# sara-nl/2D-VQ-AE-2

Measured on AMD Instinct MI355X. Metric: patches/sec (VQAE.forward: encoder -> VQ -> decoder), higher is better.
Workload: dtype f32; 1 GPU; BASELINE configs[1] (cfg B): batch 256/GPU of 256x256x3 fp32 -> 32x32 codes, K=256, D=128, full forward; global_batch=256, parallelism=patch-sharded x1

## Files before the change

2d-vq-ae-2_amd/csrc/conv_wino43.hip:

```cpp
#include "common.h"

namespace {

typedef float f32x16 __attribute__((ext_vector_type(16)));
typedef float f32x4 __attribute__((ext_vector_type(4)));
using vqae::elu_act;
using vqae::lds_barrier;

struct W43K {
    const float* __restrict__ t1;
    const float* __restrict__ U;
    const float* __restrict__ w3;
    const float* __restrict__ w1n;
    float* xio;
    float* y2;
    int H, M;
    int stag, first_gen;
    float act_a, act_b, t_scale, t_b4, n_b1a, n_b1b, n_b2a, n_b2b;
};

template <int C_> struct W43Cfg {
    static constexpr int C = C_;
    static constexpr int W = C >= 128 ? 32 : (C == 64 ? 64 : 128);
    static constexpr int NT = C == 256 ? 512 : 256;
    static constexpr int NWV = NT / 64;
    static constexpr int NS = C / 32;
    static constexpr int TG = NWV / NS;
    static constexpr int TILES = 16 * TG;
    static constexpr int TC = W / 4;
    static constexpr int PXH = 4 * W;
    static constexpr int C4 = C / 4;
    static constexpr int RP = NT / C4;
    static constexpr int LDT = C + 4;
    static constexpr int KG = C / 16;
    static constexpr int KS = C / 8;
    static constexpr int NI = C >= 64 ? 2 : 1;
    static constexpr int WN = C / (32 * NI);
    static constexpr int MI = PXH / ((NWV / WN) * 32);
    static constexpr int V_BYTES = 6 * TILES * LDT * 4, T_BYTES = PXH * LDT * 4;
    static constexpr int LDS_BYTES = V_BYTES > T_BYTES ? V_BYTES : T_BYTES;
    static_assert(TILES == 2 * TC && RP == TC && PXH / RP == 16 && MI * NI == 4, "geometry");
};
#ifndef W43_RD
#define W43_RD 4
#endif
#ifndef W43_NRES0
#define W43_NRES0 4
#endif
#ifndef W43_EARLY
#define W43_EARLY 1
#endif
constexpr int EARLY = W43_EARLY;
constexpr int RD = W43_RD;
constexpr int RT = 3;

__device__ __forceinline__ f32x4 fma4(const f32x4& a, float s, const f32x4& c) {
    return __builtin_elementwise_fma(a, f32x4{s, s, s, s}, c);
}

__device__ __forceinline__ f32x4 ldg(const float* sbase, unsigned voff_bytes) {
    return *reinterpret_cast<const f32x4*>(reinterpret_cast<const char*>(sbase) + voff_bytes);
}

#ifdef W43_TRACE
__device__ unsigned long long* g_w43_trace = nullptr;
#define STAMP(i) do { if (TAIL == 2 && lane == 0 && g_w43_trace) g_w43_trace[((int64_t)blockIdx.x * 8 + wave) * 64 + (i)] = __builtin_amdgcn_s_memtime(); } while (0)
#else
#define STAMP(i) do {} while (0)
#endif

template <int N> struct IC { static constexpr int value = N; };

template <int C, int TAIL>
__global__ __launch_bounds__((W43Cfg<C>::NT), (W43Cfg<C>::NT == 512 ? 1 : 2))
void wino43_trunk_kernel(const W43K p) {
    using K = W43Cfg<C>;
    constexpr int W = K::W, LDT = K::LDT, KG = K::KG, KS = K::KS, TILES = K::TILES, TC = K::TC, NS = K::NS, C4 = K::C4, RP = K::RP;
    constexpr int MI = K::MI, NI = K::NI, WN = K::WN;
    extern __shared__ __attribute__((aligned(16))) float lds[];
    const int tid = threadIdx.x;
    const int lane = tid & 63;
    const int wave = __builtin_amdgcn_readfirstlane(tid >> 6);
    const int li = lane & 15, q = lane >> 4;
    const int ns = wave % NS, tg = wave / NS;

    if (p.stag > 0 && (int)blockIdx.x < p.first_gen) {
        const unsigned slot = __builtin_amdgcn_s_getreg((3 << 11) | (0 << 6) | 4);
        if (slot & 1) for (int i = 0; i < p.stag; ++i) __builtin_amdgcn_s_sleep(16);
    }
#ifdef W43_TRACE
    if (TAIL == 2 && lane == 0 && g_w43_trace) {
        const unsigned hw = __builtin_amdgcn_s_getreg((15 << 11) | (0 << 6) | 4);
        const unsigned xcc = __builtin_amdgcn_s_getreg((3 << 11) | (0 << 6) | 20);
        g_w43_trace[((int64_t)blockIdx.x * 8 + wave) * 64 + 63] = ((unsigned long long)xcc << 32) | hw;
    }
#endif
    STAMP(0);
    int tile_m;
    {
        const int nwg = gridDim.x, bid = blockIdx.x;
        const int qq = nwg >> 3, r = nwg & 7, xcd = bid & 7;
        tile_m = (xcd < r ? xcd * (qq + 1) : r * (qq + 1) + (xcd - r) * qq) + (bid >> 3);
    }
    const int tpi = p.H / 8;
    const int img = tile_m / tpi;
    const int row0 = 8 * (tile_m - img * tpi);
    const float* const xim = p.t1 + (int64_t)img * p.H * W * C;

    const int cg = tid % C4, tj = tid / C4;
    unsigned coff[6];
    int roff[2][6];
#pragma unroll
    for (int j = 0; j < 6; ++j) coff[j] = (unsigned)((((4 * tj - 1 + j) & (W - 1)) * C + 4 * cg) * 4);
#pragma unroll
    for (int s = 0; s < 2; ++s)
#pragma unroll
        for (int i = 0; i < 6; ++i) {
            int r = row0 + 4 * s - 1 + i;
            r = r < 0 ? r + p.H : (r >= p.H ? r - p.H : r);
            roff[s][i] = r * W * C;
        }

    f32x4 d[2][4][2];
    f32x4 w[6];
    auto issue = [&](auto kind_c, int k) __attribute__((always_inline)) {
        constexpr int KIND = decltype(kind_c)::value;
        const int s = k / 3, cp = k % 3, bf = k & 1;
#pragma unroll
        for (int i = 0; i < (KIND == 1 ? 4 : 3); ++i) {
            const int row = KIND == 0 ? 2 * i : (KIND == 5 ? 2 * i + 1 : i + 1);
#pragma unroll
            for (int jj = 0; jj < 2; ++jj)
#ifdef W43_DBG_NOLOAD
                d[bf][i][jj] = f32x4{1.f, 2.f, (float)i, (float)tid};
#else
                d[bf][i][jj] = ldg(xim + roff[s][row], coff[2 * cp + jj]);
#endif
        }
    };
    auto combine = [&](auto kind_c, int k, float c1, float c2, float c3) __attribute__((always_inline)) {
        constexpr int KIND = decltype(kind_c)::value;
        const int cp = k % 3, bf = k & 1;
#pragma unroll
        for (int jj = 0; jj < 2; ++jj) {
            if (KIND == 1) w[2 * cp + jj] = fma4(d[bf][0][jj], c1, fma4(d[bf][1][jj], c2, fma4(d[bf][2][jj], c3, d[bf][3][jj])));
            else w[2 * cp + jj] = fma4(d[bf][0][jj], 4.f, fma4(d[bf][1][jj], -5.f, d[bf][2][jj]));
        }
    };
    auto columns = [&](int s) __attribute__((always_inline)) {
        float* const dst = lds + (s * TC + tj) * LDT + 4 * cg;
        const f32x4 t1 = fma4(w[2], -4.f, w[4]), t2 = fma4(w[1], -4.f, w[3]);
        const f32x4 t3 = w[4] - w[2], t4 = w[3] - w[1];
        *reinterpret_cast<f32x4*>(dst + 0 * TILES * LDT) = fma4(w[0], 4.f, fma4(w[2], -5.f, w[4]));
        *reinterpret_cast<f32x4*>(dst + 1 * TILES * LDT) = t1 + t2;
        *reinterpret_cast<f32x4*>(dst + 2 * TILES * LDT) = t1 - t2;
        *reinterpret_cast<f32x4*>(dst + 3 * TILES * LDT) = fma4(t4, 2.f, t3);
        *reinterpret_cast<f32x4*>(dst + 4 * TILES * LDT) = fma4(t4, -2.f, t3);
        *reinterpret_cast<f32x4*>(dst + 5 * TILES * LDT) = fma4(w[1], 4.f, fma4(w[3], -5.f, w[5]));
    };

    const float* const ub = p.U + ns * (KG * 512);
    const unsigned wl = 16u * lane;
    const float* const bfrag = lds + (16 * tg + li) * LDT + 4 * q;

    f32x4 Y[4][4][2];
#pragma unroll
    for (int a = 0; a < 4; ++a)
#pragma unroll
        for (int b = 0; b < 4; ++b) { Y[a][b][0] = f32x4{0.f, 0.f, 0.f, 0.f}; Y[a][b][1] = f32x4{0.f, 0.f, 0.f, 0.f}; }

    auto pass = [&](auto kind_c, auto next_c, int xi, float c1, float c2, float c3, float a1, float a2, float a3) __attribute__((always_inline)) {
        constexpr int KIND = decltype(kind_c)::value;
        constexpr int NEXT = decltype(next_c)::value;
        __builtin_amdgcn_sched_barrier(0);
#if defined(W43_PRIO) && W43_PRIO == 1
        __builtin_amdgcn_s_setprio(3);
#elif defined(W43_PRIO) && W43_PRIO == 2
        __builtin_amdgcn_s_setprio(0);
#endif
#pragma unroll
        for (int j = 0; j < 6; ++j) asm volatile("" : "+v"(coff[j]));
        if (EARLY < 1) issue(kind_c, 0);
#ifdef W43_SERIAL
#pragma unroll
        for (int k = 0; k < 6; ++k) {
            if (k > 0) issue(kind_c, k);
            combine(kind_c, k, c1, c2, c3);
            if (k % 3 == 2) columns(k / 3);
            __builtin_amdgcn_sched_barrier(0);
        }
#else
        if (EARLY < 2) issue(kind_c, 1);
#pragma unroll
        for (int k = 0; k < 6; ++k) {
            combine(kind_c, k, c1, c2, c3);
            if (k % 3 == 2) columns(k / 3);
            if (k + 2 < 6) issue(kind_c, k + 2);
        }
#endif
        __builtin_amdgcn_sched_barrier(0);
        int64_t uoff = (int64_t)xi * 6 * (C * C);
        asm volatile("" : "+s"(uoff));
        const float* const ux = ub + uoff;
#define WB(s) (((s) / KG) * (C * C) + 512 * ((s) % KG))
        f32x4 wq[RD][2];
#pragma unroll
        for (int s = 0; s < RD; ++s) {
            wq[s][0] = ldg(ux + WB(s), wl);
            wq[s][1] = ldg(ux + WB(s) + 256, wl);
        }
        STAMP(1 + 5 * xi);
#if defined(W43_PRIO) && W43_PRIO == 1
        __builtin_amdgcn_s_setprio(0);
#elif defined(W43_PRIO) && W43_PRIO == 2
        __builtin_amdgcn_s_setprio(3);
#endif
        lds_barrier();
        STAMP(2 + 5 * xi);
        f32x4 Z[4][2];
#pragma unroll
        for (int b = 0; b < 4; ++b) { Z[b][0] = f32x4{0.f, 0.f, 0.f, 0.f}; Z[b][1] = f32x4{0.f, 0.f, 0.f, 0.f}; }
        f32x4 acc[2][2];
        f32x4 bq[2];
        bq[0] = *reinterpret_cast<const f32x4*>(bfrag);
#pragma unroll
        for (int nu = 0; nu < 6; ++nu) {
            const int st = nu & 1;
            acc[st][0] = f32x4{0.f, 0.f, 0.f, 0.f};
            acc[st][1] = f32x4{0.f, 0.f, 0.f, 0.f};
#pragma unroll
            for (int kg = 0; kg < KG; ++kg) {
                const int s = KG * nu + kg;
                if (s + 1 < 6 * KG)
                    bq[(s + 1) & 1] = *reinterpret_cast<const f32x4*>(bfrag + ((s + 1) / KG) * TILES * LDT + 16 * ((s + 1) % KG));
                const f32x4 wa = wq[s % RD][0], wb = wq[s % RD][1];
                if (s + RD < 6 * KG) {
                    wq[s % RD][0] = ldg(ux + WB(s + RD), wl);
                    wq[s % RD][1] = ldg(ux + WB(s + RD) + 256, wl);
                }
#pragma unroll
                for (int j = 0; j < 4; ++j) {
                    acc[st][0] = __builtin_amdgcn_mfma_f32_16x16x4f32(wa[j], bq[s & 1][j], acc[st][0], 0, 0, 0);
                    acc[st][1] = __builtin_amdgcn_mfma_f32_16x16x4f32(wb[j], bq[s & 1][j], acc[st][1], 0, 0, 0);
#ifdef W43_ALT
                    __builtin_amdgcn_sched_barrier(0);
#endif
                }
                __builtin_amdgcn_sched_barrier(0);
            }
#pragma unroll
            for (int bl = 0; bl < 2; ++bl) {
                if (nu == 0) Z[0][bl] = Z[0][bl] + acc[0][bl];
                if (nu == 2) {
                    const f32x4 sm = acc[1][bl] + acc[0][bl], df = acc[1][bl] - acc[0][bl];
                    Z[0][bl] = Z[0][bl] + sm; Z[2][bl] = Z[2][bl] + sm;
                    Z[1][bl] = Z[1][bl] + df; Z[3][bl] = Z[3][bl] + df;
                }
                if (nu == 4) {
                    const f32x4 sm = acc[1][bl] + acc[0][bl], df = acc[1][bl] - acc[0][bl];
                    Z[0][bl] = Z[0][bl] + sm; Z[2][bl] = fma4(sm, 4.f, Z[2][bl]);
                    Z[1][bl] = fma4(df, 2.f, Z[1][bl]); Z[3][bl] = fma4(df, 8.f, Z[3][bl]);
                }
                if (nu == 5) Z[3][bl] = Z[3][bl] + acc[1][bl];
            }
            if (nu == 0 || nu == 2 || nu == 4)
                asm volatile("" : "+v"(Z[0][0]), "+v"(Z[0][1]), "+v"(Z[1][0]), "+v"(Z[1][1]), "+v"(Z[2][0]), "+v"(Z[2][1]), "+v"(Z[3][0]), "+v"(Z[3][1]));
        }
#undef WB
        STAMP(3 + 5 * xi);
        __builtin_amdgcn_sched_barrier(0);
        if constexpr (NEXT == 9) {
#pragma unroll
            for (int k = 0; k < EARLY; ++k)
#pragma unroll
                for (int i = 0; i < 4; ++i) {
                    const int ro = xi < 4 ? roff[0][i + 1] : roff[0][i < 3 ? 2 * i + 1 : 5];
#pragma unroll
                    for (int jj = 0; jj < 2; ++jj) d[k & 1][i][jj] = ldg(xim + ro, coff[2 * k + jj]);
                }
        } else {
            if constexpr (NEXT >= 0 && EARLY >= 1) issue(next_c, 0);
            if constexpr (NEXT >= 0 && EARLY >= 2) issue(next_c, 1);
        }
#pragma unroll
        for (int b = 0; b < 4; ++b)
#pragma unroll
            for (int bl = 0; bl < 2; ++bl) {
                if (KIND == 0) Y[0][b][bl] = Y[0][b][bl] + Z[b][bl];
                else if (KIND == 5) Y[3][b][bl] = Y[3][b][bl] + Z[b][bl];
                else {
                    Y[0][b][bl] = Y[0][b][bl] + Z[b][bl];
                    Y[1][b][bl] = fma4(Z[b][bl], a1, Y[1][b][bl]);
                    Y[2][b][bl] = fma4(Z[b][bl], a2, Y[2][b][bl]);
                    Y[3][b][bl] = fma4(Z[b][bl], a3, Y[3][b][bl]);
                }
            }
#ifdef W43_PIN_Y
#pragma unroll
        for (int a = 0; a < 4; ++a)
#pragma unroll
            for (int b = 0; b < 4; ++b) asm volatile("" : "+v"(Y[a][b][0]), "+v"(Y[a][b][1]));
#endif
        STAMP(4 + 5 * xi);
        lds_barrier();
        STAMP(5 + 5 * xi);
    };

    if (EARLY >= 1) issue(IC<0>{}, 0);
    if (EARLY >= 2) issue(IC<0>{}, 1);
    pass(IC<0>{}, IC<1>{}, 0, 0.f, 0.f, 0.f, 0.f, 0.f, 0.f);
#pragma unroll 1
    for (int xi = 1; xi <= 4; ++xi) {
        const float sg = (xi & 1) ? 1.f : -1.f;
        const bool lo = xi <= 2;
        const float c1 = lo ? -4.f * sg : -2.f * sg, c2 = lo ? -4.f : -1.f, c3 = lo ? sg : 2.f * sg;
        const float a1 = lo ? sg : 2.f * sg, a2 = lo ? 1.f : 4.f, a3 = lo ? sg : 8.f * sg;
        pass(IC<1>{}, IC<9>{}, xi, c1, c2, c3, a1, a2, a3);
    }
    pass(IC<5>{}, IC<-1>{}, 5, 0.f, 0.f, 0.f, 0.f, 0.f, 0.f);

    float* const T = lds;
    const int li32 = lane & 31, hh = lane >> 5;
    const int wm = wave / WN, wn = wave % WN;
    const int tj0 = tj;
    float* const trow = T + tj0 * LDT + 4 * cg;
    const int ty = (16 * tg + li) / TC, tx = (16 * tg + li) % TC;
    f32x4 bt[RT][NI];
    auto tail_prefetch = [&](const float* __restrict__ wsrc) __attribute__((always_inline)) {
        const float* b0 = wsrc + (wn * NI) * (KS * 256);
#pragma unroll
        for (int u = 0; u < RT; ++u)
#pragma unroll
            for (int ni = 0; ni < NI; ++ni) bt[u][ni] = ldg(b0 + ni * (KS * 256) + 256 * u, wl);
    };
    f32x16 acc[MI][NI];
    auto gemm_tail = [&](const float* __restrict__ wsrc) __attribute__((always_inline)) {
#pragma unroll
        for (int mi = 0; mi < MI; ++mi)
#pragma unroll
            for (int ni = 0; ni < NI; ++ni)
#pragma unroll
                for (int r = 0; r < 16; ++r) acc[mi][ni][r] = 0.f;
        const float* a0 = T + (wm * MI * 32 + li32) * LDT + 4 * hh;
        const float* b0 = wsrc + (wn * NI) * (KS * 256);
        f32x4 a[2][MI];
#pragma unroll
        for (int mi = 0; mi < MI; ++mi) a[0][mi] = *reinterpret_cast<const f32x4*>(a0 + mi * 32 * LDT);
#pragma unroll
        for (int ks = 0; ks < KS; ++ks) {
            if (ks + 1 < KS) {
#pragma unroll
                for (int mi = 0; mi < MI; ++mi) a[(ks + 1) & 1][mi] = *reinterpret_cast<const f32x4*>(a0 + mi * 32 * LDT + 8 * (ks + 1));
            }
            f32x4 bc[NI];
#pragma unroll
            for (int ni = 0; ni < NI; ++ni) bc[ni] = bt[ks % RT][ni];
            if (ks + RT < KS) {
#pragma unroll
                for (int ni = 0; ni < NI; ++ni) bt[ks % RT][ni] = ldg(b0 + ni * (KS * 256) + 256 * (ks + RT), wl);
            }
#pragma unroll
            for (int r = 0; r < 4; ++r)
#pragma unroll
                for (int mi = 0; mi < MI; ++mi)
#pragma unroll
                    for (int ni = 0; ni < NI; ++ni)
                        acc[mi][ni] = __builtin_amdgcn_mfma_f32_32x32x2f32(bc[ni][r], a[ks & 1][mi][r], acc[mi][ni], 0, 0, 0);
            __builtin_amdgcn_sched_barrier(0);
        }
    };
    auto acc_to_lds = [&]() __attribute__((always_inline)) {
#pragma unroll
        for (int ni = 0; ni < NI; ++ni)
#pragma unroll
            for (int mi = 0; mi < MI; ++mi)
#pragma unroll
                for (int g = 0; g < 4; ++g) {
                    f32x4 o;
#pragma unroll
                    for (int e = 0; e < 4; ++e) o[e] = acc[mi][ni][4 * g + e];
                    *reinterpret_cast<f32x4*>(T + (wm * MI * 32 + mi * 32 + li32) * LDT + (wn * NI + ni) * 32 + 8 * g + 4 * hh) = o;
                }
    };

#pragma unroll
    for (int hf = 0; hf < 2; ++hf) {
#pragma unroll
        for (int a2 = 0; a2 < 2; ++a2)
#pragma unroll
            for (int b = 0; b < 4; ++b)
#pragma unroll
                for (int bl = 0; bl < 2; ++bl) {
                    f32x4 o;
#pragma unroll
                    for (int e = 0; e < 4; ++e) o[e] = elu_act(Y[2 * hf + a2][b][bl][e] + p.act_a) + p.act_b;
                    *reinterpret_cast<f32x4*>(T + ((2 * ty + a2) * W + 4 * tx + b) * LDT + 32 * ns + 16 * bl + 4 * q) = o;
                }
        tail_prefetch(p.w3);
        const int64_t pixb = ((int64_t)img * p.H + row0 + 2 * hf) * W + tj0;
        float* xr[4];
#pragma unroll
        for (int r = 0; r < 4; ++r) xr[r] = p.xio + (pixb + (int64_t)(4 * (r >> 1) + (r & 1)) * W) * C + 4 * cg;
        f32x4 res[16];
        constexpr int NRES0 = W43_NRES0;
#pragma unroll
        for (int i = 0; i < (hf == 0 ? NRES0 : 16); ++i) res[i] = __builtin_nontemporal_load(reinterpret_cast<const f32x4*>(xr[(RP * i) / W] + ((RP * i) % W) * C));
        STAMP(31 + 8 * hf);
        lds_barrier();
        STAMP(32 + 8 * hf);
        gemm_tail(p.w3);
        STAMP(33 + 8 * hf);
        if (hf == 0) {
#pragma unroll
            for (int i = NRES0; i < 16; ++i) res[i] = __builtin_nontemporal_load(reinterpret_cast<const f32x4*>(xr[(RP * i) / W] + ((RP * i) % W) * C));
        }
        if (TAIL == 2) tail_prefetch(p.w1n);
        lds_barrier();
        acc_to_lds();
        lds_barrier();
        STAMP(34 + 8 * hf);
#pragma unroll
        for (int i = 0; i < 16; ++i) {
            f32x4 t = *reinterpret_cast<const f32x4*>(trow + RP * i * LDT);
            t = t * p.t_scale;
            t = t + p.t_b4;
            t = t + res[i];
            __builtin_nontemporal_store(t, reinterpret_cast<f32x4*>(xr[(RP * i) / W] + ((RP * i) % W) * C));
            if (TAIL == 2) {
#pragma unroll
                for (int e = 0; e < 4; ++e) t[e] = elu_act(t[e] + p.n_b1a) + p.n_b1b;
                *reinterpret_cast<f32x4*>(trow + RP * i * LDT) = t;
            }
        }
        STAMP(35 + 8 * hf);
        if constexpr (TAIL == 2) {
            lds_barrier();
            gemm_tail(p.w1n);
            STAMP(36 + 8 * hf);
            lds_barrier();
            acc_to_lds();
            lds_barrier();
            float* const y0 = p.y2 + (xr[0] - p.xio);
#pragma unroll
            for (int i = 0; i < 16; ++i) {
                f32x4 t = *reinterpret_cast<const f32x4*>(trow + RP * i * LDT);
#pragma unroll
                for (int e = 0; e < 4; ++e) t[e] = elu_act(t[e] + p.n_b2a) + p.n_b2b;
                const int r = (RP * i) / W;
                __builtin_nontemporal_store(t, reinterpret_cast<f32x4*>(y0 + ((4 * (r >> 1) + (r & 1)) * W + (RP * i) % W) * C));
            }
        }
        STAMP(37 + 8 * hf);
        if (hf == 0) lds_barrier();
        STAMP(38 + 8 * hf);
    }
}

__global__ void wino43_weight_kernel(const float* __restrict__ w, int c, float* __restrict__ U) {
    const int i = blockIdx.x * blockDim.x + threadIdx.x;
    if (i >= c * c) return;
    const double G[6][3] = {{0.25, 0, 0}, {-1.0 / 6, -1.0 / 6, -1.0 / 6}, {-1.0 / 6, 1.0 / 6, -1.0 / 6},
                            {1.0 / 24, 1.0 / 12, 1.0 / 6}, {1.0 / 24, -1.0 / 12, 1.0 / 6}, {0, 0, 1}};
    double g[3][3], t[6][3];
    for (int a = 0; a < 3; ++a)
        for (int b = 0; b < 3; ++b) g[a][b] = (double)w[(int64_t)i * 9 + a * 3 + b];
    for (int x = 0; x < 6; ++x)
        for (int b = 0; b < 3; ++b) t[x][b] = G[x][0] * g[0][b] + G[x][1] * g[1][b] + G[x][2] * g[2][b];
    const int n = i / c, k = i % c;
    const int64_t fo = ((((int64_t)(n >> 5) * (c / 16) + (k >> 4)) * 2 + ((n >> 4) & 1)) * 64 + ((k >> 2) & 3) * 16 + (n & 15)) * 4 + (k & 3);
    const int64_t cc = (int64_t)c * c;
    for (int x = 0; x < 6; ++x)
        for (int y = 0; y < 6; ++y)
            U[(x * 6 + y) * cc + fo] = (float)(t[x][0] * G[y][0] + t[x][1] * G[y][1] + t[x][2] * G[y][2]);
}

}

namespace vqae {

bool wino43_supported(int c, int h, int w, int dtype) {
    static const bool c32 = getenv("VQAE_WINO43_C32") && atoi(getenv("VQAE_WINO43_C32"));
    const bool cw = (c == 256 && w == 32) || (c == 128 && w == 32) || (c == 64 && w == 64) || (c32 && c == 32 && w == 128);
    return dtype == VQAE_DT_F32 && cw && h >= 8 && h % 8 == 0;
}
bool wino43_enabled() {
    const char* e = getenv("VQAE_WINO43");
    return !(e && !atoi(e));
}

size_t wino43_weight_floats(int c) { return (size_t)36 * c * c; }

int wino43_transform_weight(const float* w_oihw_dev, int c, float* U_dev, hipStream_t stream) {
    VQAE_REQUIRE(c == 256 || c == 128 || c == 64 || c == 32, VQAE_ERR_UNSUPPORTED, "wino43_transform_weight: C = %d", c);
    wino43_weight_kernel<<<(unsigned)ceil_div(c * c, 256), 256, 0, stream>>>(w_oihw_dev, c, U_dev);
    VQAE_LAUNCH_CHECK();
    return VQAE_OK;
}

template <int C>
static int launch_w43(W43K& k, int64_t M, bool chain, hipStream_t stream) {
    using K = W43Cfg<C>;
    static bool attr_set = false;
    static int pad = 0;
    if (!attr_set) {
#ifdef W43_TRACE
        pad = getenv("VQAE_W43_LDS_PAD") ? atoi(getenv("VQAE_W43_LDS_PAD")) : 0;
#endif
        VQAE_HIP_CHECK(hipFuncSetAttribute((const void*)wino43_trunk_kernel<C, 1>, hipFuncAttributeMaxDynamicSharedMemorySize, K::LDS_BYTES + pad));
        VQAE_HIP_CHECK(hipFuncSetAttribute((const void*)wino43_trunk_kernel<C, 2>, hipFuncAttributeMaxDynamicSharedMemorySize, K::LDS_BYTES + pad));
        attr_set = true;
    }
    const unsigned grid = (unsigned)(M / (8 * K::W));
    const double flops = 2.0 * (double)M * C * (2.25 * C + C + (chain ? C : 0));
    ProfScope prof(C >= 128 ? PROF_CONV3X3_TRUNK : PROF_NONE, stream, flops);
    if (chain) wino43_trunk_kernel<C, 2><<<grid, K::NT, K::LDS_BYTES + pad, stream>>>(k);
    else wino43_trunk_kernel<C, 1><<<grid, K::NT, K::LDS_BYTES + pad, stream>>>(k);
    prof.done();
    VQAE_LAUNCH_CHECK();
    return VQAE_OK;
}

int wino43_trunk_tail(const float* t1, const float* U, const float* w3, float act_a, float act_b, float t_scale, float t_b4,
                      float* xio, const float* w1n, float n_b1a, float n_b1b, float n_b2a, float n_b2b, float* t1_next,
                      int batch, int h, int w, int c, hipStream_t stream) {
    if (batch == 0) return VQAE_OK;
    VQAE_REQUIRE(t1 && U && w3 && xio && (!w1n || t1_next), VQAE_ERR_INVALID, "wino43_trunk_tail: null pointer");
    VQAE_REQUIRE(wino43_supported(c, h, w, VQAE_DT_F32), VQAE_ERR_UNSUPPORTED, "wino43_trunk_tail: C = %d, H = %d, W = %d", c, h, w);
    const int64_t M = (int64_t)batch * h * w;
    VQAE_REQUIRE(M < (1ll << 31) - 1024, VQAE_ERR_UNSUPPORTED, "wino43_trunk_tail: too many pixels");
    W43K k;
    memset(&k, 0, sizeof(k));
    k.t1 = t1; k.U = U; k.w3 = w3; k.w1n = w1n; k.xio = xio; k.y2 = t1_next;
    k.H = h; k.M = (int)M;
    k.act_a = act_a; k.act_b = act_b; k.t_scale = t_scale; k.t_b4 = t_b4;
    k.n_b1a = n_b1a; k.n_b1b = n_b1b; k.n_b2a = n_b2a; k.n_b2b = n_b2b;
    static const int stag = getenv("VQAE_W43_STAG") ? atoi(getenv("VQAE_W43_STAG")) : 0;
    k.stag = stag; k.first_gen = 512;
    switch (c) {
        case 256: return launch_w43<256>(k, M, w1n != nullptr, stream);
        case 128: return launch_w43<128>(k, M, w1n != nullptr, stream);
        case 64: return launch_w43<64>(k, M, w1n != nullptr, stream);
        default: return launch_w43<32>(k, M, w1n != nullptr, stream);
    }
}

}

#ifdef W43_TRACE
extern "C" int vqae_debug_w43_trace(void* dev_buf) {
    return hipMemcpyToSymbol(HIP_SYMBOL(g_w43_trace), &dev_buf, sizeof(dev_buf)) == hipSuccess ? 0 : -3;
}
#endif
```

2d-vq-ae-2_amd/csrc/handle.hip:

```cpp
#include "common.h"

#include <algorithm>
#include <cmath>
#include <cstdlib>
#include <string>
#include <unordered_map>
#include <vector>

namespace vqae {
char* last_error_buf() {
    static thread_local char buf[512] = {0};
    return buf;
}
int conv_trunk_tail(const vqae_conv_args* a, const float* t1, const float* w2, const float* w3, float t_scale,
                    float t_b4, float* xio, const float* w1n, float n_b1a, float n_b1b, float n_b2a, float n_b2b,
                    float* t1_next, hipStream_t stream);
bool wino_trunk_supported(int c, int h, int w, int dtype);
size_t wino_weight_floats(int c);
int wino_transform_weight(const float* w_oihw_dev, int c, int dtype, float* U_dev, hipStream_t stream);
int wino_frag_weight(const float* w_packed_dev, int c, int sk, float* out_dev, hipStream_t stream);
int conv_tail_kslice(int dtype, int cin);
bool wino43_supported(int c, int h, int w, int dtype);
bool wino43_enabled();
size_t wino43_weight_floats(int c);
int wino43_transform_weight(const float* w_oihw_dev, int c, float* U_dev, hipStream_t stream);
int wino43_trunk_tail(const float* t1, const float* U, const float* w3, float act_a, float act_b, float t_scale, float t_b4,
                      float* xio, const float* w1n, float n_b1a, float n_b1b, float n_b2a, float n_b2b, float* t1_next,
                      int batch, int h, int w, int c, hipStream_t stream);
int wino_trunk_tail(const float* t1, const float* U, const float* w3, float act_a, float act_b, float t_scale, float t_b4,
                    float* xio, const float* w1n, float n_b1a, float n_b1b, float n_b2a, float n_b2b, float* t1_next,
                    int batch, int h, int w, int c, int dtype, hipStream_t stream);
bool trunk16_supported(int c, int h, int w, int dtype);
size_t trunk16_weight_bytes(int c, int taps);
int trunk16_pack_weight(const float* w_packed_dev, int c, int taps, int dtype, void* out_dev, hipStream_t stream);
int trunk16_round_pack(const float* src, void* dst, int64_t n, int dtype, hipStream_t stream);
bool trunk16_head_supported(int c, int64_t m, int dtype);
int trunk16_head(const float* x, const void* w1f, float b1a, float b1b, float b2a, float b2b, void* t1, int64_t m, int c,
                 int dtype, bool out32, hipStream_t stream);
bool stem16_supported(int c0, int h, int w, int dtype);
size_t stem16_weight_bytes(int cin);
int stem16_pack_weight(const float* w_dev, int n_out, int cin, int dtype, void* out_dev, hipStream_t stream);
int istem16(const void* x, int x_kind, const float* mean255, const float* inv_std255, const void* wf, const float* bias, int B,
            int H, int W, int c0, float* y, int dtype, hipStream_t stream);
int ostem16(const float* x, const void* wf, const float* bias, int B, int H, int W, int c, float* y, int y_nchw, int dtype,
            hipStream_t stream);
bool same8_16_supported(int c, int h, int w, int dtype);
int same8_16_block(const float* x, float* y, const float* w1_packed, const void* w2h, const void* w3h, int B, int H, int W,
                   const float* scalars8, int dtype, hipStream_t stream);
bool same16_16_supported(int c, int h, int w, int dtype);
int same16_16_block(const float* x, float* y, const void* w1h, const void* w2h, const void* w3h, int B, int H, int W, int c,
                    const float* scalars8, int dtype, hipStream_t stream);
bool up16_supported(int c, int h, int w, int dtype);
int up16_block(const float* x, const float* t1, const void* w2h, const void* w3h, const void* wskh, int B, int H, int W, int c,
               float b3a, float b3b, float scale, float b4, float b1c, float b1d, int dtype, float* y, hipStream_t stream);
int trunk16_block(const void* t1, const void* w2f, const void* w3f, float act_a, float act_b, float t_scale, float t_b4,
                  float* xio, const void* w1nf, float n_b1a, float n_b1b, float n_b2a, float n_b2b, void* t1_next,
                  int batch, int h, int w, int c, int dtype, hipStream_t stream);
bool fixup_conv1_supported(int c, int64_t m);
int fixup_conv1(const float* x, const float* w1f, float pa, float pb, float aa, float ab, float* y, int64_t m, int c,
                hipStream_t stream);
bool down_block_supported(int cin, int h, int w);
int frag_weight_rect(const float* w_packed_dev, int n_rows, int K, float* out_dev, hipStream_t stream);
bool down16_supported(int cin, int h, int w);
size_t down16_weight_bytes(int n_rows, int K);
int down16_pack_weight(const float* w_packed_dev, int n_rows, int K, int dtype, void* out_dev, hipStream_t stream);
int down16_block(const float* x, const void* w1h, const void* w2h, const void* w3h, const void* wskh, int B, int H, int W,
                 int cin, const float* scalars10, int dtype, float* y, hipStream_t stream);
int down_block(const float* x, const float* w1f, const float* w2f, const float* w3f, const float* wskf, int B, int H, int W,
               int cin, const float* scalars10, int dtype, float* y, hipStream_t stream);
bool up_tail_supported(int cb, int co);
int up_tail(const float* q, const float* s, const float* w3_packed, int B, int H, int W, int cb, int co, float b3a, float b3b,
            float scale, float b4, float* y, hipStream_t stream);
int conv3x3_direct(const void* x, int x_kind, const float* mean255, const float* inv_std255, const float* w,
                   const float* bias, int B, int H, int W, int cin, int cout, float* y, int y_nchw, int dt,
                   hipStream_t stream);
}

namespace vqae {
ProfState& prof_state() {
    static ProfState p;
    return p;
}
}

extern "C" int vqae_prof_begin(int kernel_class, int max_launches) {
    vqae::ProfState& p = vqae::prof_state();
    VQAE_REQUIRE(kernel_class >= 1 && kernel_class <= 3 && max_launches >= 1, VQAE_ERR_INVALID, "prof_begin: bad args");
    if (p.cap < 2 * max_launches) {
        for (int i = 0; i < p.cap; ++i) (void)hipEventDestroy(p.ev[i]);
        delete[] p.ev;
        p.ev = new hipEvent_t[2 * max_launches];
        p.cap = 0;
        for (int i = 0; i < 2 * max_launches; ++i) {
            VQAE_HIP_CHECK(hipEventCreate(&p.ev[i]));
            p.cap = i + 1;
        }
    }
    p.used = 0;
    p.work = 0.0;
    p.cls = kernel_class;
    return VQAE_OK;
}

extern "C" int vqae_prof_end(double* total_ms, int* n_launches, double* total_work) {
    vqae::ProfState& p = vqae::prof_state();
    p.cls = 0;
    double tot = 0.0;
    for (int i = 0; i + 1 < p.used; i += 2) {
        VQAE_HIP_CHECK(hipEventSynchronize(p.ev[i + 1]));
        float ms = 0.f;
        VQAE_HIP_CHECK(hipEventElapsedTime(&ms, p.ev[i], p.ev[i + 1]));
        tot += ms;
    }
    if (total_ms) *total_ms = tot;
    if (n_launches) *n_launches = p.used / 2;
    if (total_work) *total_work = p.work;
    p.used = 0;
    return VQAE_OK;
}

extern "C" const char* vqae_last_error(void) { return vqae::last_error_buf(); }
extern "C" const char* vqae_build_info(void) { return "gfx950;fp32-mfma;" __DATE__; }

namespace {

enum { MODE_SAME = 0, MODE_DOWN = 1, MODE_UP = 2 };

struct Block {
    int mode, cin, cout, br;
    float b1a, b1b, b2a, b2b, b3a, b3b, b4, scale, b1c, b1d;
    float *w1, *w2, *w3, *wskip;
    float* wU43 = nullptr;
    float* wU = nullptr;
    float *w1f = nullptr, *w3f = nullptr;
    float *w2f = nullptr, *wskf = nullptr;
    void *w1h = nullptr, *w2h = nullptr, *w3h = nullptr;
    void *dw1h = nullptr, *dw2h = nullptr, *dw3h = nullptr, *dwskh = nullptr;
    void *uw1h = nullptr, *uw2h = nullptr, *uw3h = nullptr, *uwskh = nullptr;
    void *s8w2h = nullptr, *s8w3h = nullptr;
    int kind = VQAE_BLOCK_FIXUP, hidden = 0;
    float *bv1 = nullptr, *bv2 = nullptr, *bv3 = nullptr;
    float *fc0w = nullptr, *fc0b = nullptr, *fc2w = nullptr, *fc2b = nullptr;
};

const float kMean255[3] = {0.7279f * 255.0f, 0.5955f * 255.0f, 0.7762f * 255.0f};
const float kInv255[3] = {1.0f / (0.2419f * 255.0f), 1.0f / (0.3083f * 255.0f), 1.0f / (0.1741f * 255.0f)};

}

struct vqae_handle {
    vqae_config cfg;
    int C = 0, D = 0, K = 0;
    std::vector<Block> enc, dec;
    float *stem_w = nullptr, *stem_b = nullptr, *ostem_w = nullptr, *ostem_b = nullptr;
    void *stem_wh = nullptr, *ostem_wh = nullptr;
    bool fuse_stem16 = true;
    float *embed = nullptr;
    float *pin_w = nullptr, *pin_b = nullptr, *pout_w = nullptr, *pout_b = nullptr;
    float *pin_wt = nullptr, *pout_wr = nullptr;
    bool fuse_vq = true;
    std::vector<void*> owned;
    float* buf[4] = {nullptr, nullptr, nullptr, nullptr};
    size_t buf_floats = 0;
    void* vq_ws = nullptr;
    size_t vq_ws_bytes = 0;
    float* loss_scratch = nullptr;
    int device = 0;
    bool has_encoder = false, has_decoder = false;
    bool fuse_trunk = true;
    bool t1_ready = false;
    bool up_conv_first = true;
    bool fuse_down = true;
    bool fuse_down16 = true;
    bool fuse_up16 = true;
    bool fuse_up_tail = true;
    bool use_wino = true;
    void* idx_scratch = nullptr;
    size_t idx_scratch_bytes = 0;
    float* se_ws = nullptr;
    size_t se_ws_floats = 0;
    size_t se_gate_off = 0;
};

namespace {

using TensorMap = std::unordered_map<std::string, const vqae_tensor*>;

int find(const TensorMap& tm, const std::string& name, int64_t numel, const float** out) {
    auto it = tm.find(name);
    if (it == tm.end()) return vqae::fail(VQAE_ERR_NOT_FOUND, "missing tensor '%s'", name.c_str());
    if (it->second->numel != numel)
        return vqae::fail(VQAE_ERR_INVALID, "tensor '%s' has %lld elements, expected %lld", name.c_str(),
                          (long long)it->second->numel, (long long)numel);
    *out = it->second->data;
    return VQAE_OK;
}

int dev_alloc(vqae_handle* h, size_t bytes, void** out) {
    void* p = nullptr;
    if (hipMalloc(&p, bytes ? bytes : 16) != hipSuccess)
        return vqae::fail(VQAE_ERR_NOMEM, "hipMalloc of %zu bytes failed", bytes);
    h->owned.push_back(p);
    *out = p;
    return VQAE_OK;
}

int upload(vqae_handle* h, const float* host, int64_t numel, float** out) {
    void* p;
    int rc = dev_alloc(h, (size_t)numel * 4, &p);
    if (rc) return rc;
    VQAE_HIP_CHECK(hipMemcpy(p, host, (size_t)numel * 4, hipMemcpyHostToDevice));
    *out = (float*)p;
    return VQAE_OK;
}

int upload_packed(vqae_handle* h, const float* host, int cout, int cin, int ks, float** out) {
    float* raw = nullptr;
    void* tmp = nullptr;
    const int64_t numel = (int64_t)cout * cin * ks * ks;
    if (hipMalloc(&tmp, (size_t)numel * 4) != hipSuccess) return vqae::fail(VQAE_ERR_NOMEM, "hipMalloc failed");
    raw = (float*)tmp;
    hipError_t e = hipMemcpy(raw, host, (size_t)numel * 4, hipMemcpyHostToDevice);
    void* packed = nullptr;
    int rc = (e == hipSuccess) ? dev_alloc(h, vqae_conv_packed_floats(cout, cin, ks) * 4, &packed)
                               : vqae::fail(VQAE_ERR_HIP, "hipMemcpy failed: %s", hipGetErrorString(e));
    if (rc == VQAE_OK) rc = vqae_conv_pack_weight_f32(raw, cout, cin, ks, (float*)packed, nullptr);
    if (rc == VQAE_OK) rc = vqae_round_inplace_f32((float*)packed, (int64_t)vqae_conv_packed_floats(cout, cin, ks), h->cfg.compute_dtype, nullptr);
    if (rc == VQAE_OK && hipDeviceSynchronize() != hipSuccess) rc = vqae::fail(VQAE_ERR_HIP, "pack sync failed");
    (void)hipFree(tmp);
    *out = (float*)packed;
    return rc;
}

int upload_wino(vqae_handle* h, const float* host, int c, float** out) {
    void* tmp = nullptr;
    const size_t raw = (size_t)c * c * 9 * 4;
    if (hipMalloc(&tmp, raw) != hipSuccess) return vqae::fail(VQAE_ERR_NOMEM, "hipMalloc failed");
    hipError_t e = hipMemcpy(tmp, host, raw, hipMemcpyHostToDevice);
    void* U = nullptr;
    int rc = (e == hipSuccess) ? dev_alloc(h, vqae::wino_weight_floats(c) * 4, &U)
                               : vqae::fail(VQAE_ERR_HIP, "hipMemcpy failed: %s", hipGetErrorString(e));
    if (rc == VQAE_OK) rc = vqae::wino_transform_weight((const float*)tmp, c, h->cfg.compute_dtype, (float*)U, nullptr);
    if (rc == VQAE_OK && hipDeviceSynchronize() != hipSuccess) rc = vqae::fail(VQAE_ERR_HIP, "winograd weight transform failed");
    (void)hipFree(tmp);
    *out = (float*)U;
    return rc;
}

int upload_wino43(vqae_handle* h, const float* host, int c, float** out) {
    void* tmp = nullptr;
    const size_t raw = (size_t)c * c * 9 * 4;
    if (hipMalloc(&tmp, raw) != hipSuccess) return vqae::fail(VQAE_ERR_NOMEM, "hipMalloc failed");
    hipError_t e = hipMemcpy(tmp, host, raw, hipMemcpyHostToDevice);
    void* U = nullptr;
    int rc = (e == hipSuccess) ? dev_alloc(h, vqae::wino43_weight_floats(c) * 4, &U)
                               : vqae::fail(VQAE_ERR_HIP, "hipMemcpy failed: %s", hipGetErrorString(e));
    if (rc == VQAE_OK) rc = vqae::wino43_transform_weight((const float*)tmp, c, (float*)U, nullptr);
    if (rc == VQAE_OK && hipDeviceSynchronize() != hipSuccess) rc = vqae::fail(VQAE_ERR_HIP, "winograd weight transform failed");
    (void)hipFree(tmp);
    *out = (float*)U;
    return rc;
}

int scalar(const TensorMap& tm, const std::string& name, float* out) {
    const float* p;
    int rc = find(tm, name, 1, &p);
    if (rc) return rc;
    *out = p[0];
    return VQAE_OK;
}

int load_block(vqae_handle* h, const TensorMap& tm, const std::string& pre, int mode, int cin, int cout, Block* b) {
    b->mode = mode; b->cin = cin; b->cout = cout; b->br = cin > cout ? cin : cout;
    b->w1 = b->w2 = b->w3 = b->wskip = nullptr;
    b->b1c = b->b1d = 0.f;
    int rc;
#define S_(field, nm) if ((rc = scalar(tm, pre + "." nm, &b->field))) return rc;
    S_(b1a, "bias1a") S_(b1b, "bias1b") S_(b2a, "bias2a") S_(b2b, "bias2b") S_(b3a, "bias3a") S_(b3b, "bias3b")
    S_(b4, "bias4") S_(scale, "scale")
    const int k2 = mode == MODE_SAME ? 3 : (mode == MODE_DOWN ? 2 : 1);
    const float* p;
    if ((rc = find(tm, pre + ".branch_conv1.weight", (int64_t)b->br * cin, &p))) return rc;
    if ((rc = upload_packed(h, p, b->br, cin, 1, &b->w1))) return rc;
    if ((rc = find(tm, pre + ".branch_conv2.weight", (int64_t)b->br * b->br * k2 * k2, &p))) return rc;
    if ((rc = upload_packed(h, p, b->br, b->br, k2, &b->w2))) return rc;
    b->wU = b->wU43 = b->w1f = b->w3f = nullptr;
    const bool wino = mode == MODE_SAME && cout == cin && h->use_wino &&
                      (h->cfg.compute_dtype == VQAE_DT_F32 ? (cin == 256 || cin == 128 || cin == 64 || cin == 32) : cin == 32);
    if (wino && (rc = upload_wino(h, p, cin, &b->wU))) return rc;
    if (wino && h->cfg.compute_dtype == VQAE_DT_F32 && vqae::wino43_enabled() && vqae::wino43_supported(cin, 8, cin >= 128 ? 32 : (cin == 64 ? 64 : 128), VQAE_DT_F32) &&
        (rc = upload_wino43(h, p, cin, &b->wU43))) return rc;
    if ((rc = find(tm, pre + ".branch_conv3.weight", (int64_t)cout * b->br, &p))) return rc;
    if ((rc = upload_packed(h, p, cout, b->br, 1, &b->w3))) return rc;
    if (wino || (mode == MODE_SAME && (cin == 128 || cin == 64) && cout == cin)) {
        const int sk = wino ? 8 : vqae::conv_tail_kslice(h->cfg.compute_dtype, cin);
        void *f1, *f3;
        if ((rc = dev_alloc(h, (size_t)cin * cin * 4, &f1)) || (rc = dev_alloc(h, (size_t)cin * cin * 4, &f3))) return rc;
        b->w1f = (float*)f1; b->w3f = (float*)f3;
        if ((rc = vqae::wino_frag_weight(b->w1, cin, sk, b->w1f, nullptr)) || (rc = vqae::wino_frag_weight(b->w3, cin, sk, b->w3f, nullptr))) return rc;
        VQAE_HIP_CHECK(hipDeviceSynchronize());
    }
    b->w1h = b->w2h = b->w3h = nullptr;
    if (mode == MODE_SAME && cout == cin && h->cfg.compute_dtype != VQAE_DT_F32 && (cin == 16 || cin == 32 || cin == 64 || cin == 128 || cin == 256)) {
        struct { float* src; int taps; void** dst; } m[3] = {{b->w1, 1, &b->w1h}, {b->w2, 9, &b->w2h}, {b->w3, 1, &b->w3h}};
        for (auto& e : m) {
            if ((rc = dev_alloc(h, vqae::trunk16_weight_bytes(cin, e.taps), e.dst))) return rc;
            if ((rc = vqae::trunk16_pack_weight(e.src, cin, e.taps, h->cfg.compute_dtype, *e.dst, nullptr))) return rc;
        }
        VQAE_HIP_CHECK(hipDeviceSynchronize());
    }
    if (mode != MODE_SAME) {
        S_(b1c, "bias1c") S_(b1d, "bias1d")
        const int ks = mode == MODE_DOWN ? 2 : 1;
        if ((rc = find(tm, pre + ".skip_conv.weight", (int64_t)cout * cin * ks * ks, &p))) return rc;
        if ((rc = upload_packed(h, p, cout, cin, ks, &b->wskip))) return rc;
    }
    b->w2f = b->wskf = nullptr;
    if (mode == MODE_DOWN && h->fuse_down && cout == 2 * cin &&
        (cin == 16 || cin == 32 || cin == 64)) {
        struct { float* src; int K; float** dst; } m[4] = {{b->w1, cin, &b->w1f}, {b->w2, 4 * cout, &b->w2f},
                                                          {b->w3, cout, &b->w3f}, {b->wskip, 4 * cin, &b->wskf}};
        for (auto& e : m) {
            void* f;
            if ((rc = dev_alloc(h, (size_t)cout * e.K * 4, &f))) return rc;
            *e.dst = (float*)f;
            if ((rc = vqae::frag_weight_rect(e.src, cout, e.K, *e.dst, nullptr))) return rc;
        }
        VQAE_HIP_CHECK(hipDeviceSynchronize());
    }
    if (mode == MODE_DOWN && cout == 2 * cin && h->cfg.compute_dtype != VQAE_DT_F32 && h->fuse_down16 &&
        (cin == 8 || cin == 16 || cin == 32 || cin == 64)) {
        struct { float* src; int K; void** dst; } m16[4] = {{b->w1, cin, &b->dw1h}, {b->w2, 4 * cout, &b->dw2h},
                                                            {b->w3, cout, &b->dw3h}, {b->wskip, 4 * cin, &b->dwskh}};
        for (auto& e : m16) {
            if ((rc = dev_alloc(h, vqae::down16_weight_bytes(cout, e.K), e.dst))) return rc;
            if ((rc = vqae::down16_pack_weight(e.src, cout, e.K, h->cfg.compute_dtype, *e.dst, nullptr))) return rc;
        }
        VQAE_HIP_CHECK(hipDeviceSynchronize());
    }
    if (mode == MODE_SAME && cin == 8 && cout == 8 && h->cfg.compute_dtype != VQAE_DT_F32) {
        if ((rc = dev_alloc(h, vqae::down16_weight_bytes(8, 72), &b->s8w2h)) || (rc = dev_alloc(h, vqae::down16_weight_bytes(8, 8), &b->s8w3h))) return rc;
        if ((rc = vqae::down16_pack_weight(b->w2, 8, 72, h->cfg.compute_dtype, b->s8w2h, nullptr))) return rc;
        if ((rc = vqae::down16_pack_weight(b->w3, 8, 8, h->cfg.compute_dtype, b->s8w3h, nullptr))) return rc;
        VQAE_HIP_CHECK(hipDeviceSynchronize());
    }
    if (mode == MODE_UP && cin == 2 * cout && h->cfg.compute_dtype != VQAE_DT_F32 && h->fuse_up16 &&
        (cin == 16 || cin == 32 || cin == 64 || cin == 128)) {
        if ((rc = dev_alloc(h, vqae::trunk16_weight_bytes(cin, 1), &b->uw1h))) return rc;
        if ((rc = vqae::trunk16_pack_weight(b->w1, cin, 1, h->cfg.compute_dtype, b->uw1h, nullptr))) return rc;
        struct { float* src; int rows; void** dst; } mu[3] = {{b->w2, cin, &b->uw2h}, {b->w3, cout, &b->uw3h}, {b->wskip, cout, &b->uwskh}};
        for (auto& e : mu) {
            if ((rc = dev_alloc(h, vqae::down16_weight_bytes(e.rows, cin), e.dst))) return rc;
            if ((rc = vqae::down16_pack_weight(e.src, e.rows, cin, h->cfg.compute_dtype, *e.dst, nullptr))) return rc;
        }
        VQAE_HIP_CHECK(hipDeviceSynchronize());
    }
#undef S_
    return VQAE_OK;
}

int bn_fold(const TensorMap& tm, const std::string& pre, int c, float eps, std::vector<float>* g, std::vector<float>* shift) {
    const float *gamma, *beta, *mean, *var;
    int rc;
    if ((rc = find(tm, pre + ".weight", c, &gamma)) || (rc = find(tm, pre + ".bias", c, &beta)) ||
        (rc = find(tm, pre + ".running_mean", c, &mean)) || (rc = find(tm, pre + ".running_var", c, &var))) return rc;
    g->resize(c); shift->resize(c);
    for (int i = 0; i < c; ++i) {
        (*g)[i] = gamma[i] / std::sqrt(var[i] + eps);
        (*shift)[i] = beta[i] - mean[i] * (*g)[i];
    }
    return VQAE_OK;
}

int load_mbconv(vqae_handle* h, const TensorMap& tm, const std::string& pre, int mode, int cin, int cout, Block* b) {
    *b = Block();
    b->kind = VQAE_BLOCK_MBCONV;
    b->mode = mode; b->cin = cin; b->cout = cout;
    const int e = (cin > cout ? cin : cout) * h->cfg.expand_ratio;
    b->br = e;
    const int div = h->cfg.se_divisor;
    b->hidden = std::max(div, (int)(e + div / 2.0)) / div;
    VQAE_REQUIRE(e % 32 == 0 && e <= 1024, VQAE_ERR_UNSUPPORTED, "MBConv: expanded width %d must be a multiple of 32, <= 1024", e);
    const std::string br = pre + ".branch.";
    const float eps = h->cfg.bn_eps;
    std::vector<float> g, sh, w;
    const float* p;
    int rc;
    if ((rc = find(tm, br + "0.weight", (int64_t)e * cin, &p)) || (rc = bn_fold(tm, br + "1", e, eps, &g, &sh))) return rc;
    w.assign(p, p + (int64_t)e * cin);
    for (int o = 0; o < e; ++o) for (int i = 0; i < cin; ++i) w[(int64_t)o * cin + i] *= g[o];
    if ((rc = upload_packed(h, w.data(), e, cin, 1, &b->w1)) || (rc = upload(h, sh.data(), e, &b->bv1))) return rc;
    const int k2 = mode == MODE_SAME ? 3 : 2;
    if ((rc = find(tm, br + "3.weight", (int64_t)e * k2 * k2, &p)) || (rc = bn_fold(tm, br + "4", e, eps, &g, &sh))) return rc;
    w.assign((size_t)k2 * k2 * e, 0.f);
    for (int c = 0; c < e; ++c) for (int t = 0; t < k2 * k2; ++t) w[(size_t)t * e + c] = p[(size_t)c * k2 * k2 + t] * g[c];
    if ((rc = upload(h, w.data(), (int64_t)k2 * k2 * e, &b->w2)) || (rc = upload(h, sh.data(), e, &b->bv2))) return rc;
    if ((rc = find(tm, br + "6.fc.0.weight", (int64_t)b->hidden * e, &p)) || (rc = upload(h, p, (int64_t)b->hidden * e, &b->fc0w))) return rc;
    if ((rc = find(tm, br + "6.fc.0.bias", b->hidden, &p)) || (rc = upload(h, p, b->hidden, &b->fc0b))) return rc;
    if ((rc = find(tm, br + "6.fc.2.weight", (int64_t)e * b->hidden, &p)) || (rc = upload(h, p, (int64_t)e * b->hidden, &b->fc2w))) return rc;
    if ((rc = find(tm, br + "6.fc.2.bias", e, &p)) || (rc = upload(h, p, e, &b->fc2b))) return rc;
    if ((rc = find(tm, br + "7.weight", (int64_t)cout * e, &p)) || (rc = bn_fold(tm, br + "8", cout, eps, &g, &sh))) return rc;
    w.assign(p, p + (int64_t)cout * e);
    for (int o = 0; o < cout; ++o) for (int i = 0; i < e; ++i) w[(int64_t)o * e + i] *= g[o];
    if ((rc = upload_packed(h, w.data(), cout, e, 1, &b->w3)) || (rc = upload(h, sh.data(), cout, &b->bv3))) return rc;
    if (mode == MODE_DOWN) {
        if ((rc = find(tm, pre + ".skip_conv.weight", (int64_t)cout * cin * 4, &p)) || (rc = upload_packed(h, p, cout, cin, 2, &b->wskip))) return rc;
    } else if (mode == MODE_UP) {
        if ((rc = find(tm, pre + ".skip_conv.weight", (int64_t)cin * cout * 4, &p))) return rc;
        w.assign((size_t)4 * cout * cin, 0.f);
        for (int ci = 0; ci < cin; ++ci) for (int co = 0; co < cout; ++co) for (int t = 0; t < 4; ++t)
            w[((size_t)t * cout + co) * cin + ci] = p[((size_t)ci * cout + co) * 4 + t];
        if ((rc = upload_packed(h, w.data(), 4 * cout, cin, 1, &b->wskip))) return rc;
    } else if (cin != cout) {
        if ((rc = find(tm, pre + ".skip_conv.weight", (int64_t)cout * cin, &p)) || (rc = upload_packed(h, p, cout, cin, 1, &b->wskip))) return rc;
    }
    return VQAE_OK;
}

int load_any(vqae_handle* h, const TensorMap& tm, const std::string& pre, int mode, int cin, int cout, Block* b) {
    return h->cfg.block_kind == VQAE_BLOCK_MBCONV ? load_mbconv(h, tm, pre, mode, cin, cout, b)
                                                  : load_block(h, tm, pre, mode, cin, cout, b);
}

thread_local int g_dt = VQAE_DT_F32;
struct ConvCall {
    vqae_conv_args a;
    ConvCall(int B, int H, int W, int cin, int cout, int ks, int stride, int pad, int pad_mode, int dt = g_dt) {
        memset(&a, 0, sizeof(a));
        a.dtype = dt;
        a.batch = B; a.in_h = H; a.in_w = W; a.cin = cin; a.cout = cout;
        a.ksize = ks; a.stride = stride; a.pad = pad; a.pad_mode = pad_mode;
    }
    ConvCall& pre(int mode, float pa, float pb) { a.pre_mode = mode; a.pre_a = pa; a.pre_b = pb; return *this; }
    ConvCall& act(float aa, float ab) { a.has_act = 1; a.act_a = aa; a.act_b = ab; return *this; }
    ConvCall& scale_bias(float s, float b) { a.has_scale = 1; a.scale = s; a.bias_s = b; return *this; }
    ConvCall& bias(float b) { a.has_bias_s = 1; a.bias_s = b; return *this; }
};

int run_mbconv(vqae_handle* h, const Block& b, int B, int& H, int& W, hipStream_t st) {
    float *X = h->buf[0], *P = h->buf[1], *Q = h->buf[2], *R = h->buf[3];
    float* partial = h->se_ws;
    float* gate = h->se_ws + h->se_gate_off;
    const int E = b.br;
    int rc;
    const float* skip = X;
    int Ho = H, Wo = W;
    if (b.mode == MODE_DOWN) {
        ConvCall sk(B, H, W, b.cin, b.cout, 2, 2, 0, VQAE_PAD_NONE);
        if ((rc = vqae_conv2d_f32(&sk.a, X, b.wskip, nullptr, nullptr, R, st))) return rc;
        skip = R; Ho = H / 2; Wo = W / 2;
    } else if (b.mode == MODE_UP) {
        ConvCall sk(B, H, W, b.cin, 4 * b.cout, 1, 1, 0, VQAE_PAD_NONE);
        if ((rc = vqae_conv2d_f32(&sk.a, X, b.wskip, nullptr, nullptr, Q, st))) return rc;
        if ((rc = vqae_pixel_shuffle2_f32(Q, B, H, W, b.cout, R, st))) return rc;
        skip = R; Ho = 2 * H; Wo = 2 * W;
    } else if (b.wskip) {
        ConvCall sk(B, H, W, b.cin, b.cout, 1, 1, 0, VQAE_PAD_NONE);
        if ((rc = vqae_conv2d_f32(&sk.a, X, b.wskip, nullptr, nullptr, R, st))) return rc;
        skip = R;
    }
    ConvCall c1(B, H, W, b.cin, E, 1, 1, 0, VQAE_PAD_NONE);
    c1.a.has_act = VQAE_ACT_SILU;
    if ((rc = vqae_conv2d_f32(&c1.a, X, b.w1, b.bv1, nullptr, P, st))) return rc;
    const int dwm = b.mode == MODE_SAME ? VQAE_DW_SAME : (b.mode == MODE_DOWN ? VQAE_DW_DOWN : VQAE_DW_UP);
    if ((rc = vqae_dwconv_f32(P, b.w2, b.bv2, B, H, W, E, dwm, 1, Q, partial, st))) return rc;
    if ((rc = vqae_se_gate_f32(partial, B, Ho, Wo, E, b.fc0w, b.fc0b, b.hidden, b.fc2w, b.fc2b, gate, st))) return rc;
    ConvCall c3(B, Ho, Wo, E, b.cout, 1, 1, 0, VQAE_PAD_NONE);
    c3.a.pre_mode = VQAE_PRE_CHANNEL_GATE;
    float* out = skip == X ? X : R;
    if ((rc = vqae_conv2d_gated_f32(&c3.a, Q, gate, b.w3, b.bv3, skip, out, st))) return rc;
    if (out == R) std::swap(h->buf[0], h->buf[3]);
    H = Ho; W = Wo;
    return VQAE_OK;
}

int run_block(vqae_handle* h, const Block& b, const Block* next, int B, int& H, int& W, hipStream_t st) {
    if (b.kind == VQAE_BLOCK_MBCONV) return run_mbconv(h, b, B, H, W, st);
    float *X = h->buf[0], *P = h->buf[1], *Q = h->buf[2], *R = h->buf[3];
    int rc;
    if (b.mode == MODE_SAME && b.w2h && h->fuse_trunk && vqae::same16_16_supported(b.cin, H, W, g_dt)) {
        const float sc[8] = {b.b1a, b.b1b, b.b2a, b.b2b, b.b3a, b.b3b, b.b4, b.scale};
        if ((rc = vqae::same16_16_block(X, P, b.w1h, b.w2h, b.w3h, B, H, W, b.cin, sc, g_dt, st))) return rc;
        std::swap(h->buf[0], h->buf[1]);
        h->t1_ready = false;
        return VQAE_OK;
    }
    if (b.mode == MODE_SAME && b.w2h && h->fuse_trunk && vqae::trunk16_supported(b.cin, H, W, g_dt)) {
        if (!h->t1_ready && vqae::trunk16_head_supported(b.cin, (int64_t)B * H * W, g_dt)) {
            if ((rc = vqae::trunk16_head(X, b.w1h, b.b1a, b.b1b, b.b2a, b.b2b, P, (int64_t)B * H * W, b.cin, g_dt, false, st))) return rc;
        } else if (!h->t1_ready) {
            ConvCall c1(B, H, W, b.cin, b.br, 1, 1, 0, VQAE_PAD_NONE);
            c1.pre(VQAE_PRE_BIAS_ELU_BIAS, b.b1a, b.b1b).act(b.b2a, b.b2b);
            if ((rc = vqae_conv2d_f32(&c1.a, X, b.w1, nullptr, nullptr, Q, st))) return rc;
            if ((rc = vqae::trunk16_round_pack(Q, P, (int64_t)B * H * W * b.cin, g_dt, st))) return rc;
        }
        const bool chain = next && next->mode == MODE_SAME && next->cin == b.cin && next->cout == b.cin && next->w1h;
        if ((rc = vqae::trunk16_block(P, b.w2h, b.w3h, b.b3a, b.b3b, b.scale, b.b4, X, chain ? next->w1h : nullptr,
                                      chain ? next->b1a : 0.f, chain ? next->b1b : 0.f, chain ? next->b2a : 0.f,
                                      chain ? next->b2b : 0.f, chain ? Q : nullptr, B, H, W, b.cin, g_dt, st))) return rc;
        if (chain) std::swap(h->buf[1], h->buf[2]);
        h->t1_ready = chain;
        return VQAE_OK;
    }
    const bool wino = b.mode == MODE_SAME && b.wU && h->fuse_trunk && vqae::wino_trunk_supported(b.cin, H, W, g_dt);
    if (b.mode == MODE_SAME && (wino || ((b.cin == 128 || b.cin == 64) && b.cout == b.cin && h->fuse_trunk))) {
        if (!h->t1_ready) {
            const int64_t M = (int64_t)B * H * W;
            if (wino && g_dt == VQAE_DT_F32 && vqae::fixup_conv1_supported(b.cin, M)) {
                if ((rc = vqae::fixup_conv1(X, b.w1f, b.b1a, b.b1b, b.b2a, b.b2b, P, M, b.cin, st))) return rc;
            } else {
                ConvCall c1(B, H, W, b.cin, b.br, 1, 1, 0, VQAE_PAD_NONE);
                c1.pre(VQAE_PRE_BIAS_ELU_BIAS, b.b1a, b.b1b).act(b.b2a, b.b2b);
                if ((rc = vqae_conv2d_f32(&c1.a, X, b.w1, nullptr, nullptr, P, st))) return rc;
            }
        }
        const bool chain = next && next->mode == MODE_SAME && next->cin == b.cin && next->cout == b.cin && (!wino || next->w1f);
        if (wino && b.wU43 && vqae::wino43_supported(b.cin, H, W, g_dt)) {
            if ((rc = vqae::wino43_trunk_tail(P, b.wU43, b.w3f, b.b3a, b.b3b, b.scale, b.b4, X, chain ? next->w1f : nullptr,
                                              chain ? next->b1a : 0.f, chain ? next->b1b : 0.f, chain ? next->b2a : 0.f,
                                              chain ? next->b2b : 0.f, chain ? Q : nullptr, B, H, W, b.cin, st))) return rc;
            if (chain) std::swap(h->buf[1], h->buf[2]);
            h->t1_ready = chain;
            return VQAE_OK;
        }
        if (wino) {
            if ((rc = vqae::wino_trunk_tail(P, b.wU, b.w3f, b.b3a, b.b3b, b.scale, b.b4, X, chain ? next->w1f : nullptr,
                                            chain ? next->b1a : 0.f, chain ? next->b1b : 0.f, chain ? next->b2a : 0.f,
                                            chain ? next->b2b : 0.f, chain ? Q : nullptr, B, H, W, b.cin, g_dt, st))) return rc;
            if (chain) std::swap(h->buf[1], h->buf[2]);
            h->t1_ready = chain;
            return VQAE_OK;
        }
        ConvCall c2(B, H, W, b.br, b.br, 3, 1, 1, VQAE_PAD_CIRCULAR);
        c2.act(b.b3a, b.b3b);
        if ((rc = vqae::conv_trunk_tail(&c2.a, P, b.w2, b.w3f, b.scale, b.b4, X, chain ? next->w1f : nullptr,
                                        chain ? next->b1a : 0.f, chain ? next->b1b : 0.f, chain ? next->b2a : 0.f,
                                        chain ? next->b2b : 0.f, chain ? Q : nullptr, st))) return rc;
        if (chain) std::swap(h->buf[1], h->buf[2]);
        h->t1_ready = chain;
        return VQAE_OK;
    }
    h->t1_ready = false;
    if (b.mode == MODE_SAME && b.s8w2h && g_dt != VQAE_DT_F32 && vqae::same8_16_supported(b.cin, H, W, g_dt)) {
        const float sc[8] = {b.b1a, b.b1b, b.b2a, b.b2b, b.b3a, b.b3b, b.b4, b.scale};
        if ((rc = vqae::same8_16_block(X, P, b.w1, b.s8w2h, b.s8w3h, B, H, W, sc, g_dt, st))) return rc;
        std::swap(h->buf[0], h->buf[1]);
        return VQAE_OK;
    }
    if (b.mode == MODE_SAME && b.cin == b.cout && vqae_fixup_same_supported(b.cin, H, W)) {
        const float sc[8] = {b.b1a, b.b1b, b.b2a, b.b2b, b.b3a, b.b3b, b.b4, b.scale};
        if ((rc = vqae_fixup_same_block_f32(X, P, b.w1, b.w2, b.w3, B, H, W, b.cin, sc, g_dt, st))) return rc;
        std::swap(h->buf[0], h->buf[1]);
        return VQAE_OK;
    }
    if (b.mode == MODE_SAME) {
        ConvCall c1(B, H, W, b.cin, b.br, 1, 1, 0, VQAE_PAD_NONE);
        c1.pre(VQAE_PRE_BIAS_ELU_BIAS, b.b1a, b.b1b).act(b.b2a, b.b2b);
        if ((rc = vqae_conv2d_f32(&c1.a, X, b.w1, nullptr, nullptr, P, st))) return rc;
        ConvCall c2(B, H, W, b.br, b.br, 3, 1, 1, VQAE_PAD_CIRCULAR);
        c2.act(b.b3a, b.b3b);
        if ((rc = vqae_conv2d_f32(&c2.a, P, b.w2, nullptr, nullptr, Q, st))) return rc;
        ConvCall c3(B, H, W, b.br, b.cout, 1, 1, 0, VQAE_PAD_NONE);
        c3.scale_bias(b.scale, b.b4);
        return vqae_conv2d_f32(&c3.a, Q, b.w3, nullptr, X, X, st);
    }
    if (b.mode == MODE_DOWN && b.dw2h && g_dt != VQAE_DT_F32 && vqae::down16_supported(b.cin, H, W)) {
        const float sc[10] = {b.b1a, b.b1b, b.b2a, b.b2b, b.b3a, b.b3b, b.b4, b.scale, b.b1c, b.b1d};
        if ((rc = vqae::down16_block(X, b.dw1h, b.dw2h, b.dw3h, b.dwskh, B, H, W, b.cin, sc, g_dt, R, st))) return rc;
        H /= 2; W /= 2;
        std::swap(h->buf[0], h->buf[3]);
        return VQAE_OK;
    }
    if (b.mode == MODE_DOWN && b.w2f && vqae::down_block_supported(b.cin, H, W)) {
        const float sc[10] = {b.b1a, b.b1b, b.b2a, b.b2b, b.b3a, b.b3b, b.b4, b.scale, b.b1c, b.b1d};
        if ((rc = vqae::down_block(X, b.w1f, b.w2f, b.w3f, b.wskf, B, H, W, b.cin, sc, g_dt, R, st))) return rc;
        H /= 2; W /= 2;
        std::swap(h->buf[0], h->buf[3]);
        return VQAE_OK;
    }
    if (b.mode == MODE_DOWN) {
        ConvCall sk(B, H, W, b.cin, b.cout, 2, 2, 0, VQAE_PAD_NONE);
        sk.pre(VQAE_PRE_BIAS, b.b1c, 0.f).bias(b.b1d);
        if ((rc = vqae_conv2d_f32(&sk.a, X, b.wskip, nullptr, nullptr, R, st))) return rc;
        ConvCall c1(B, H, W, b.cin, b.br, 1, 1, 0, VQAE_PAD_NONE);
        c1.pre(VQAE_PRE_BIAS_ELU_BIAS, b.b1a, b.b1b).act(b.b2a, b.b2b);
        if ((rc = vqae_conv2d_f32(&c1.a, X, b.w1, nullptr, nullptr, P, st))) return rc;
        ConvCall c2(B, H, W, b.br, b.br, 2, 2, 0, VQAE_PAD_NONE);
        c2.act(b.b3a, b.b3b);
        if ((rc = vqae_conv2d_f32(&c2.a, P, b.w2, nullptr, nullptr, Q, st))) return rc;
        H /= 2; W /= 2;
        ConvCall c3(B, H, W, b.br, b.cout, 1, 1, 0, VQAE_PAD_NONE);
        c3.scale_bias(b.scale, b.b4);
        if ((rc = vqae_conv2d_f32(&c3.a, Q, b.w3, nullptr, R, R, st))) return rc;
        std::swap(h->buf[0], h->buf[3]);
        return VQAE_OK;
    }
    if (g_dt == VQAE_DT_F32 && h->up_conv_first) {
        ConvCall sk(B, H, W, b.cin, b.cout, 1, 1, 0, VQAE_PAD_NONE);
        sk.pre(VQAE_PRE_BIAS, b.b1c, 0.f).bias(b.b1d);
        if ((rc = vqae_conv2d_f32(&sk.a, X, b.wskip, nullptr, nullptr, Q, st))) return rc;
        if (h->fuse_up_tail && vqae::up_tail_supported(b.br, b.cout)) {
            ConvCall c1(B, H, W, b.cin, b.br, 1, 1, 0, VQAE_PAD_NONE);
            c1.pre(VQAE_PRE_BIAS_ELU_BIAS, b.b1a, b.b1b).act(b.b2a, b.b2b);
            if ((rc = vqae_conv2d_f32(&c1.a, X, b.w1, nullptr, nullptr, P, st))) return rc;
            ConvCall c2(B, H, W, b.br, b.br, 1, 1, 0, VQAE_PAD_NONE);
            if ((rc = vqae_conv2d_f32(&c2.a, P, b.w2, nullptr, nullptr, R, st))) return rc;
            if ((rc = vqae::up_tail(R, Q, b.w3, B, H, W, b.br, b.cout, b.b3a, b.b3b, b.scale, b.b4, X, st))) return rc;
            H *= 2; W *= 2;
            return VQAE_OK;
        }
        if ((rc = vqae_bicubic_up2_f32(Q, B, H, W, b.cout, 0.f, R, st))) return rc;
        ConvCall c1(B, H, W, b.cin, b.br, 1, 1, 0, VQAE_PAD_NONE);
        c1.pre(VQAE_PRE_BIAS_ELU_BIAS, b.b1a, b.b1b).act(b.b2a, b.b2b);
        if ((rc = vqae_conv2d_f32(&c1.a, X, b.w1, nullptr, nullptr, P, st))) return rc;
        ConvCall c2(B, H, W, b.br, b.br, 1, 1, 0, VQAE_PAD_NONE);
        if ((rc = vqae_conv2d_f32(&c2.a, P, b.w2, nullptr, nullptr, Q, st))) return rc;
        if ((rc = vqae_bicubic_up2_f32(Q, B, H, W, b.br, 0.f, P, st))) return rc;
        H *= 2; W *= 2;
        ConvCall c3(B, H, W, b.br, b.cout, 1, 1, 0, VQAE_PAD_NONE);
        c3.pre(VQAE_PRE_BIAS_ELU_BIAS, b.b3a, b.b3b).scale_bias(b.scale, b.b4);
        if ((rc = vqae_conv2d_f32(&c3.a, P, b.w3, nullptr, R, R, st))) return rc;
        std::swap(h->buf[0], h->buf[3]);
        return VQAE_OK;
    }
    if (b.uw2h && vqae::up16_supported(b.cin, H, W, g_dt) && vqae::trunk16_head_supported(b.cin, (int64_t)B * H * W, g_dt)) {
        if ((rc = vqae::trunk16_head(X, b.uw1h, b.b1a, b.b1b, b.b2a, b.b2b, Q, (int64_t)B * H * W, b.cin, g_dt, true, st))) return rc;
        if ((rc = vqae::up16_block(X, Q, b.uw2h, b.uw3h, b.uwskh, B, H, W, b.cin, b.b3a, b.b3b, b.scale, b.b4, b.b1c, b.b1d, g_dt, R, st))) return rc;
        H *= 2; W *= 2;
        std::swap(h->buf[0], h->buf[3]);
        return VQAE_OK;
    }
    if ((rc = vqae_bicubic_up2_f32(X, B, H, W, b.cin, b.b1c, P, st))) return rc;
    ConvCall sk(B, 2 * H, 2 * W, b.cin, b.cout, 1, 1, 0, VQAE_PAD_NONE);
    sk.bias(b.b1d);
    if ((rc = vqae_conv2d_f32(&sk.a, P, b.wskip, nullptr, nullptr, R, st))) return rc;
    ConvCall c1(B, H, W, b.cin, b.br, 1, 1, 0, VQAE_PAD_NONE);
    c1.pre(VQAE_PRE_BIAS_ELU_BIAS, b.b1a, b.b1b).act(b.b2a, b.b2b);
    if ((rc = vqae_conv2d_f32(&c1.a, X, b.w1, nullptr, nullptr, Q, st))) return rc;
    if ((rc = vqae_bicubic_up2_f32(Q, B, H, W, b.br, 0.f, P, st))) return rc;
    H *= 2; W *= 2;
    ConvCall c2(B, H, W, b.br, b.br, 1, 1, 0, VQAE_PAD_NONE);
    c2.act(b.b3a, b.b3b);
    if ((rc = vqae_conv2d_f32(&c2.a, P, b.w2, nullptr, nullptr, Q, st))) return rc;
    ConvCall c3(B, H, W, b.br, b.cout, 1, 1, 0, VQAE_PAD_NONE);
    c3.scale_bias(b.scale, b.b4);
    if ((rc = vqae_conv2d_f32(&c3.a, Q, b.w3, nullptr, R, R, st))) return rc;
    std::swap(h->buf[0], h->buf[3]);
    return VQAE_OK;
}

size_t max_floats_per_patch(const vqae_handle* h, int in_h, int in_w) {
    const size_t widen = h->cfg.block_kind == VQAE_BLOCK_MBCONV ? (size_t)h->cfg.expand_ratio : 1;
    size_t full = (size_t)in_h * in_w * (size_t)(2 * h->cfg.stem) * widen;
    size_t lat = (size_t)(in_h >> h->cfg.n_down) * (in_w >> h->cfg.n_down) * (size_t)h->C * widen;
    return full > lat ? full : lat;
}

int ensure_bufs(vqae_handle* h, size_t need) {
    if (need > h->buf_floats) {
        VQAE_HIP_CHECK(hipDeviceSynchronize());
        for (int i = 0; i < 4; ++i) {
            if (h->buf[i]) (void)hipFree(h->buf[i]);
            h->buf[i] = nullptr;
        }
        h->buf_floats = 0;
        for (int i = 0; i < 4; ++i)
            if (hipMalloc((void**)&h->buf[i], need * sizeof(float)) != hipSuccess)
                return vqae::fail(VQAE_ERR_NOMEM, "workspace hipMalloc of %zu bytes failed", need * sizeof(float));
        h->buf_floats = need;
    }
    return VQAE_OK;
}

int ensure_workspace(vqae_handle* h, int B, int in_h, int in_w) {
    int rc = ensure_bufs(h, max_floats_per_patch(h, in_h, in_w) * (size_t)(B > 0 ? B : 1));
    if (rc) return rc;
    const int64_t rows = (int64_t)B * (in_h >> h->cfg.n_down) * (in_w >> h->cfg.n_down);
    size_t vq_need = vqae_vq_workspace_bytes(rows, h->K, h->D);
    if (h->D == 8) vq_need = std::max(vq_need, vqae_vq_projected_workspace_bytes(rows));
    if (vq_need > h->vq_ws_bytes) {
        VQAE_HIP_CHECK(hipDeviceSynchronize());
        if (h->vq_ws) (void)hipFree(h->vq_ws);
        h->vq_ws = nullptr; h->vq_ws_bytes = 0;
        if (hipMalloc(&h->vq_ws, vq_need) != hipSuccess)
            return vqae::fail(VQAE_ERR_NOMEM, "vq workspace hipMalloc of %zu bytes failed", vq_need);
        h->vq_ws_bytes = vq_need;
    }
    if (h->cfg.block_kind == VQAE_BLOCK_MBCONV) {
        const int e_max = 2 * h->cfg.stem * h->cfg.expand_ratio, e_lat = h->C * h->cfg.expand_ratio;
        size_t part = vqae_dw_partial_floats(B, in_h, in_w, e_max);
        const size_t part_lat = vqae_dw_partial_floats(B, in_h >> h->cfg.n_down, in_w >> h->cfg.n_down, e_lat);
        if (part_lat > part) part = part_lat;
        for (int l = 1; l < h->cfg.n_down; ++l) {
            const size_t pl = vqae_dw_partial_floats(B, in_h >> l, in_w >> l, (2 * h->cfg.stem << l) * h->cfg.expand_ratio);
            if (pl > part) part = pl;
        }
        const size_t gate_floats = (size_t)(B > 0 ? B : 1) * (size_t)(e_lat > e_max ? e_lat : e_max);
        const size_t need_se = (size_t)vqae::round_up((int64_t)part, 64) + gate_floats;
        if (need_se > h->se_ws_floats) {
            VQAE_HIP_CHECK(hipDeviceSynchronize());
            if (h->se_ws) (void)hipFree(h->se_ws);
            h->se_ws = nullptr; h->se_ws_floats = 0;
            if (hipMalloc((void**)&h->se_ws, need_se * 4) != hipSuccess)
                return vqae::fail(VQAE_ERR_NOMEM, "SE workspace hipMalloc of %zu bytes failed", need_se * 4);
            h->se_ws_floats = need_se;
        }
        h->se_gate_off = h->se_ws_floats - gate_floats;
    }
    const size_t idx_need = (size_t)vqae::round_up(rows * 4, 256);
    if (idx_need > h->idx_scratch_bytes) {
        VQAE_HIP_CHECK(hipDeviceSynchronize());
        if (h->idx_scratch) (void)hipFree(h->idx_scratch);
        h->idx_scratch = nullptr; h->idx_scratch_bytes = 0;
        if (hipMalloc(&h->idx_scratch, idx_need) != hipSuccess)
            return vqae::fail(VQAE_ERR_NOMEM, "idx scratch hipMalloc of %zu bytes failed", idx_need);
        h->idx_scratch_bytes = idx_need;
    }
    return VQAE_OK;
}

int check_device(const vqae_handle* h) {
    int dev = -1;
    VQAE_HIP_CHECK(hipGetDevice(&dev));
    VQAE_REQUIRE(dev == h->device, VQAE_ERR_INVALID, "handle was created on HIP device %d but the current device is %d", h->device, dev);
    return VQAE_OK;
}

int check_geometry(const vqae_handle* h, int B, int in_h, int in_w) {
    const int f = 1 << h->cfg.n_down;
    if (int rc = check_device(h)) return rc;
    VQAE_REQUIRE(B >= 0, VQAE_ERR_INVALID, "negative batch");
    VQAE_REQUIRE(in_h >= f && in_w >= f && in_h % f == 0 && in_w % f == 0, VQAE_ERR_INVALID,
                 "input %dx%d must be a positive multiple of 2^n_down = %d", in_h, in_w, f);
    return VQAE_OK;
}

int run_encoder_convs(vqae_handle* h, const void* x, int x_kind, int B, int in_h, int in_w, int* zh, int* zw,
                      hipStream_t st) {
    int rc;
    if (h->stem_wh && vqae::stem16_supported(h->cfg.stem, in_h, in_w, g_dt)) {
        if ((rc = vqae::istem16(x, x_kind, kMean255, kInv255, h->stem_wh, h->stem_b, B, in_h, in_w, h->cfg.stem, h->buf[0], g_dt, st))) return rc;
    } else if ((rc = vqae::conv3x3_direct(x, x_kind, kMean255, kInv255, h->stem_w, h->stem_b, B, in_h, in_w,
                                          h->cfg.in_channels, h->cfg.stem, h->buf[0], 0, g_dt, st))) return rc;
    int H = in_h, W = in_w;
    h->t1_ready = false;
    for (size_t i = 0; i < h->enc.size(); ++i)
        if ((rc = run_block(h, h->enc[i], i + 1 < h->enc.size() ? &h->enc[i + 1] : nullptr, B, H, W, st))) return rc;
    *zh = H; *zw = W;
    return VQAE_OK;
}

int run_vq(vqae_handle* h, int B, int zh, int zw, void* idx, int idx_dtype, float* loss, hipStream_t st) {
    const int64_t rows = (int64_t)B * zh * zw;
    int rc;
    if (h->cfg.projection_dim == 8 && h->fuse_vq && h->pin_wt) {
        if ((rc = vqae_vq_projected_f32(h->buf[0], h->pin_wt, h->pin_b, h->embed, h->pout_wr, h->pout_b, rows, h->C, h->D, h->K,
                                        h->cfg.commitment_cost, g_dt, idx, idx_dtype, h->buf[1], nullptr, loss, nullptr,
                                        h->vq_ws, st))) return rc;
        std::swap(h->buf[0], h->buf[1]);
        return VQAE_OK;
    }
    if (h->cfg.projection_dim > 0) {
        ConvCall pin(B, zh, zw, h->C, h->D, 1, 1, 0, VQAE_PAD_NONE);
        if ((rc = vqae_conv2d_f32(&pin.a, h->buf[0], h->pin_w, h->pin_b, nullptr, h->buf[1], st))) return rc;
        if ((rc = vqae_vq_forward_f32(h->buf[1], h->embed, rows, h->K, h->D, h->cfg.commitment_cost, idx, idx_dtype,
                                      h->buf[2], loss, nullptr, h->vq_ws, st))) return rc;
        ConvCall pout(B, zh, zw, h->D, h->C, 1, 1, 0, VQAE_PAD_NONE);
        return vqae_conv2d_f32(&pout.a, h->buf[2], h->pout_w, h->pout_b, nullptr, h->buf[0], st);
    }
    if ((rc = vqae_vq_forward_f32(h->buf[0], h->embed, rows, h->K, h->D, h->cfg.commitment_cost, idx, idx_dtype,
                                  h->buf[1], loss, nullptr, h->vq_ws, st))) return rc;
    std::swap(h->buf[0], h->buf[1]);
    return VQAE_OK;
}

int run_decoder_convs(vqae_handle* h, int B, int qh, int qw, int layout, float* out, hipStream_t st) {
    int H = qh, W = qw, rc;
    h->t1_ready = false;
    for (size_t i = 0; i < h->dec.size(); ++i)
        if ((rc = run_block(h, h->dec[i], i + 1 < h->dec.size() ? &h->dec[i + 1] : nullptr, B, H, W, st))) return rc;
    if (h->ostem_wh && vqae::stem16_supported(h->cfg.stem, H, W, g_dt))
        return vqae::ostem16(h->buf[0], h->ostem_wh, h->ostem_b, B, H, W, h->cfg.stem, out, layout == VQAE_LAYOUT_NCHW ? 1 : 0, g_dt, st);
    return vqae::conv3x3_direct(h->buf[0], 0, nullptr, nullptr, h->ostem_w, h->ostem_b, B, H, W, h->cfg.stem,
                                h->cfg.in_channels, out, layout == VQAE_LAYOUT_NCHW ? 1 : 0, g_dt, st);
}

int export_q(vqae_handle* h, int B, int zh, int zw, int layout, float* q, hipStream_t st) {
    if (!q) return VQAE_OK;
    if (layout == VQAE_LAYOUT_NCHW) return vqae_nhwc_to_nchw_f32(h->buf[0], B, h->C, zh, zw, q, st);
    VQAE_HIP_CHECK(hipMemcpyAsync(q, h->buf[0], (size_t)B * zh * zw * h->C * 4, hipMemcpyDeviceToDevice, st));
    return VQAE_OK;
}

}

extern "C" int vqae_create(const vqae_config* cfg, const vqae_tensor* tensors, int n_tensors, vqae_handle** out) {
    VQAE_REQUIRE(cfg && tensors && out, VQAE_ERR_INVALID, "vqae_create: null pointer");
    VQAE_REQUIRE(cfg->in_channels == 3, VQAE_ERR_UNSUPPORTED, "in_channels %d (only 3)", cfg->in_channels);
    VQAE_REQUIRE(cfg->stem >= 4 && cfg->stem % 4 == 0 && cfg->stem <= 64, VQAE_ERR_UNSUPPORTED, "stem %d", cfg->stem);
    VQAE_REQUIRE(cfg->stem % 8 == 0, VQAE_ERR_UNSUPPORTED, "stem %d must be a multiple of 8", cfg->stem);
    VQAE_REQUIRE(cfg->n_down >= 1 && cfg->n_down <= 6 && cfg->n_pre >= 0 && cfg->n_post >= 0 && cfg->n_enc >= 0,
                 VQAE_ERR_INVALID, "bad depth parameters");
    VQAE_REQUIRE(cfg->num_embeddings >= 1 && cfg->num_embeddings <= 65536, VQAE_ERR_UNSUPPORTED, "num_embeddings %d",
                 cfg->num_embeddings);
    VQAE_REQUIRE(cfg->projection_dim == 0 || (cfg->projection_dim % 8 == 0), VQAE_ERR_UNSUPPORTED,
                 "projection_dim %d must be 0 or a multiple of 8", cfg->projection_dim);
    VQAE_REQUIRE(cfg->compute_dtype >= VQAE_DT_F32 && cfg->compute_dtype <= VQAE_DT_F16, VQAE_ERR_INVALID,
                 "compute_dtype %d", cfg->compute_dtype);
    VQAE_REQUIRE(cfg->block_kind == VQAE_BLOCK_FIXUP || cfg->block_kind == VQAE_BLOCK_MBCONV, VQAE_ERR_INVALID,
                 "block_kind %d", cfg->block_kind);
    if (cfg->block_kind == VQAE_BLOCK_MBCONV) {
        VQAE_REQUIRE(cfg->compute_dtype == VQAE_DT_F32, VQAE_ERR_UNSUPPORTED, "MBConv blocks run in fp32 only");
        VQAE_REQUIRE(cfg->expand_ratio >= 1 && cfg->se_divisor >= 1 && cfg->bn_eps > 0.f, VQAE_ERR_INVALID,
                     "MBConv: expand_ratio %d, se_divisor %d, bn_eps %g", cfg->expand_ratio, cfg->se_divisor, (double)cfg->bn_eps);
    }
    TensorMap tm;
    for (int i = 0; i < n_tensors; ++i) tm[tensors[i].name] = &tensors[i];

    vqae_handle* h = new vqae_handle();
    h->cfg = *cfg;
    if (hipGetDevice(&h->device) != hipSuccess) { delete h; return vqae::fail(VQAE_ERR_HIP, "hipGetDevice failed"); }
    h->fuse_trunk = !(getenv("VQAE_NO_TRUNK_FUSION") && atoi(getenv("VQAE_NO_TRUNK_FUSION")));
    h->up_conv_first = !(getenv("VQAE_NO_UP_REORDER") && atoi(getenv("VQAE_NO_UP_REORDER")));
    h->use_wino = !(getenv("VQAE_NO_WINOGRAD") && atoi(getenv("VQAE_NO_WINOGRAD")));
    h->fuse_up_tail = !(getenv("VQAE_NO_UP_TAIL_FUSION") && atoi(getenv("VQAE_NO_UP_TAIL_FUSION")));
    h->fuse_down = !(getenv("VQAE_NO_DOWN_FUSION") && atoi(getenv("VQAE_NO_DOWN_FUSION")));
    h->fuse_down16 = !(getenv("VQAE_NO_DOWN16") && atoi(getenv("VQAE_NO_DOWN16")));
    h->fuse_up16 = !(getenv("VQAE_NO_UP16") && atoi(getenv("VQAE_NO_UP16")));
    h->fuse_stem16 = !(getenv("VQAE_NO_STEM16") && atoi(getenv("VQAE_NO_STEM16")));
    h->fuse_vq = !(getenv("VQAE_NO_VQ_FUSION") && atoi(getenv("VQAE_NO_VQ_FUSION")));
    h->C = cfg->stem << cfg->n_down;
    h->D = cfg->projection_dim > 0 ? cfg->projection_dim : h->C;
    h->K = cfg->num_embeddings;
    int rc = VQAE_OK;
    const float* p;
    auto bail = [&](int code) { vqae_destroy(h); return code; };

    const bool has_enc = tm.count("encoder.in_stem.weight") > 0;
    const bool has_dec = tm.count("decoder.out_stem.weight") > 0;
    if (!has_enc && !has_dec) return bail(vqae::fail(VQAE_ERR_NOT_FOUND, "neither encoder.* nor decoder.* tensors given"));
    h->has_encoder = has_enc;
    h->has_decoder = has_dec;
    int c = cfg->stem << cfg->n_down;
    const std::string vq = "encoder.vq_layers.0.";

    if (has_enc) {
        if ((rc = find(tm, "encoder.in_stem.weight", (int64_t)cfg->stem * 3 * 9, &p)) || (rc = upload(h, p, (int64_t)cfg->stem * 27, &h->stem_w))) return bail(rc);
        if ((rc = find(tm, "encoder.in_stem.bias", cfg->stem, &p)) || (rc = upload(h, p, cfg->stem, &h->stem_b))) return bail(rc);
        if (cfg->compute_dtype != VQAE_DT_F32 && h->fuse_stem16 && cfg->in_channels == 3 && (cfg->stem == 8 || cfg->stem == 16 || cfg->stem == 32)) {
            if ((rc = dev_alloc(h, vqae::stem16_weight_bytes(3), &h->stem_wh))) return bail(rc);
            if ((rc = vqae::stem16_pack_weight(h->stem_w, cfg->stem, 3, cfg->compute_dtype, h->stem_wh, nullptr))) return bail(rc);
        }
        c = cfg->stem;
        for (int lvl = 0; lvl < cfg->n_down; ++lvl) {
            const std::string base = "encoder.down_layers.0.layers." + std::to_string(lvl) + ".layers.";
            int bi = 0;
            Block b;
            for (int i = 0; i < cfg->n_pre; ++i, ++bi) {
                if ((rc = load_any(h, tm, base + std::to_string(bi), MODE_SAME, c, c, &b))) return bail(rc);
                h->enc.push_back(b);
            }
            if ((rc = load_any(h, tm, base + std::to_string(bi), MODE_DOWN, c, 2 * c, &b))) return bail(rc);
            h->enc.push_back(b); ++bi;
            for (int i = 0; i < cfg->n_post; ++i, ++bi) {
                if ((rc = load_any(h, tm, base + std::to_string(bi), MODE_SAME, 2 * c, 2 * c, &b))) return bail(rc);
                h->enc.push_back(b);
            }
            c *= 2;
        }
        for (int i = 0; i < cfg->n_enc; ++i) {
            Block b;
            if ((rc = load_any(h, tm, "encoder.pre_enc_layers.0." + std::to_string(i), MODE_SAME, c, c, &b))) return bail(rc);
            h->enc.push_back(b);
        }
    }
    if (has_enc || tm.count(vq + "embed")) {
        if ((rc = find(tm, vq + "embed", (int64_t)h->K * h->D, &p)) || (rc = upload(h, p, (int64_t)h->K * h->D, &h->embed))) return bail(rc);
        if (cfg->projection_dim > 0) {
            if ((rc = find(tm, vq + "proj_in.weight", (int64_t)h->D * h->C, &p)) || (rc = upload_packed(h, p, h->D, h->C, 1, &h->pin_w))) return bail(rc);
            if ((rc = find(tm, vq + "proj_in.bias", h->D, &p)) || (rc = upload(h, p, h->D, &h->pin_b))) return bail(rc);
            if ((rc = vqae_round_inplace_f32(h->pin_b, h->D, cfg->compute_dtype, nullptr))) return bail(rc);
            if ((rc = find(tm, vq + "proj_out.weight", (int64_t)h->C * h->D, &p)) || (rc = upload_packed(h, p, h->C, h->D, 1, &h->pout_w))) return bail(rc);
            if ((rc = find(tm, vq + "proj_out.bias", h->C, &p)) || (rc = upload(h, p, h->C, &h->pout_b))) return bail(rc);
            if ((rc = vqae_round_inplace_f32(h->pout_b, h->C, cfg->compute_dtype, nullptr))) return bail(rc);
            if (h->D == 8) {
                std::vector<float> wt((size_t)h->C * 8);
                const float* pi = tm.at(vq + "proj_in.weight")->data;
                for (int j = 0; j < 8; ++j) for (int cc = 0; cc < h->C; ++cc) wt[(size_t)cc * 8 + j] = pi[(size_t)j * h->C + cc];
                if ((rc = upload(h, wt.data(), (int64_t)h->C * 8, &h->pin_wt)) ||
                    (rc = upload(h, tm.at(vq + "proj_out.weight")->data, (int64_t)h->C * 8, &h->pout_wr))) return bail(rc);
                if ((rc = vqae_round_inplace_f32(h->pin_wt, (int64_t)h->C * 8, cfg->compute_dtype, nullptr)) ||
                    (rc = vqae_round_inplace_f32(h->pout_wr, (int64_t)h->C * 8, cfg->compute_dtype, nullptr))) return bail(rc);
            }
        }
    }
    if (has_dec) {
        if ((rc = find(tm, "decoder.out_stem.weight", (int64_t)3 * cfg->stem * 9, &p)) || (rc = upload(h, p, (int64_t)cfg->stem * 27, &h->ostem_w))) return bail(rc);
        if ((rc = find(tm, "decoder.out_stem.bias", 3, &p)) || (rc = upload(h, p, 3, &h->ostem_b))) return bail(rc);
        if (cfg->compute_dtype != VQAE_DT_F32 && h->fuse_stem16 && cfg->in_channels == 3 && (cfg->stem == 8 || cfg->stem == 16 || cfg->stem == 32)) {
            if ((rc = dev_alloc(h, vqae::stem16_weight_bytes(cfg->stem), &h->ostem_wh))) return bail(rc);
            if ((rc = vqae::stem16_pack_weight(h->ostem_w, 3, cfg->stem, cfg->compute_dtype, h->ostem_wh, nullptr))) return bail(rc);
        }
        c = cfg->stem << cfg->n_down;
        for (int i = 0; i < cfg->n_enc; ++i) {
            Block b;
            if ((rc = load_any(h, tm, "decoder.post_enc_layers.0." + std::to_string(i), MODE_SAME, c, c, &b))) return bail(rc);
            h->dec.push_back(b);
        }
        for (int lvl = 0; lvl < cfg->n_down; ++lvl) {
            const std::string base = "decoder.up_layers.0.layers." + std::to_string(lvl) + ".layers.";
            int bi = 0;
            Block b;
            for (int i = 0; i < cfg->n_pre; ++i, ++bi) {
                if ((rc = load_any(h, tm, base + std::to_string(bi), MODE_SAME, c, c, &b))) return bail(rc);
                h->dec.push_back(b);
            }
            if ((rc = load_any(h, tm, base + std::to_string(bi), MODE_UP, c, c / 2, &b))) return bail(rc);
            h->dec.push_back(b); ++bi;
            for (int i = 0; i < cfg->n_post; ++i, ++bi) {
                if ((rc = load_any(h, tm, base + std::to_string(bi), MODE_SAME, c / 2, c / 2, &b))) return bail(rc);
                h->dec.push_back(b);
            }
            c /= 2;
        }
    }
    void* ls = nullptr;
    if ((rc = dev_alloc(h, 256, &ls))) return bail(rc);
    h->loss_scratch = (float*)ls;
    *out = h;
    return VQAE_OK;
}

extern "C" void vqae_destroy(vqae_handle* h) {
    if (!h) return;
    (void)hipDeviceSynchronize();
    for (void* p : h->owned) (void)hipFree(p);
    for (int i = 0; i < 4; ++i)
        if (h->buf[i]) (void)hipFree(h->buf[i]);
    if (h->vq_ws) (void)hipFree(h->vq_ws);
    if (h->idx_scratch) (void)hipFree(h->idx_scratch);
    if (h->se_ws) (void)hipFree(h->se_ws);
    delete h;
}

extern "C" int vqae_reserve(vqae_handle* h, int max_batch, int in_h, int in_w) {
    VQAE_REQUIRE(h, VQAE_ERR_INVALID, "null handle");
    int rc = check_geometry(h, max_batch, in_h, in_w);
    if (rc) return rc;
    return ensure_workspace(h, max_batch, in_h, in_w);
}

extern "C" int vqae_set_codebook(vqae_handle* h, const float* embed_host) {
    VQAE_REQUIRE(h && embed_host && h->embed, VQAE_ERR_INVALID, "set_codebook: null pointer / handle has no codebook");
    VQAE_HIP_CHECK(hipDeviceSynchronize());
    VQAE_HIP_CHECK(hipMemcpy(h->embed, embed_host, (size_t)h->K * h->D * 4, hipMemcpyHostToDevice));
    return VQAE_OK;
}

static int encode_impl(vqae_handle* h, const void* x, int x_kind, int B, int in_h, int in_w, void* idx, int idx_dtype,
                       float* q, int q_layout, float* loss, hipStream_t st) {
    if (h) g_dt = h->cfg.compute_dtype;
    VQAE_REQUIRE(h && x && idx, VQAE_ERR_INVALID, "vqae_encode: null pointer");
    VQAE_REQUIRE(h->has_encoder, VQAE_ERR_INVALID, "vqae_encode: handle was created without encoder.* tensors");
    int rc = check_geometry(h, B, in_h, in_w);
    if (rc) return rc;
    if (B == 0) return VQAE_OK;
    if ((rc = ensure_workspace(h, B, in_h, in_w))) return rc;
    int zh, zw;
    if ((rc = run_encoder_convs(h, x, x_kind, B, in_h, in_w, &zh, &zw, st))) return rc;
    if ((rc = run_vq(h, B, zh, zw, idx, idx_dtype, loss, st))) return rc;
    return export_q(h, B, zh, zw, q_layout, q, st);
}

extern "C" int vqae_encode(vqae_handle* h, const float* x, int B, int in_h, int in_w, int layout, void* idx,
                           int idx_dtype, float* q, float* loss, void* stream) {
    return encode_impl(h, x, layout == VQAE_LAYOUT_NCHW ? 1 : 0, B, in_h, in_w, idx, idx_dtype, q, layout, loss,
                       (hipStream_t)stream);
}

extern "C" int vqae_encode_u8(vqae_handle* h, const uint8_t* x, int B, int in_h, int in_w, void* idx, int idx_dtype,
                              float* q, int q_layout, float* loss, void* stream) {
    return encode_impl(h, x, 2, B, in_h, in_w, idx, idx_dtype, q, q_layout, loss, (hipStream_t)stream);
}

extern "C" int vqae_encode_features(vqae_handle* h, const float* x, int B, int in_h, int in_w, int layout, float* z,
                                    void* stream) {
    if (h) g_dt = h->cfg.compute_dtype;
    hipStream_t st = (hipStream_t)stream;
    VQAE_REQUIRE(h && x && z, VQAE_ERR_INVALID, "vqae_encode_features: null pointer");
    VQAE_REQUIRE(h->has_encoder, VQAE_ERR_INVALID, "vqae_encode_features: handle has no encoder");
    int rc = check_geometry(h, B, in_h, in_w);
    if (rc) return rc;
    if (B == 0) return VQAE_OK;
    if ((rc = ensure_workspace(h, B, in_h, in_w))) return rc;
    int zh, zw;
    if ((rc = run_encoder_convs(h, x, layout == VQAE_LAYOUT_NCHW ? 1 : 0, B, in_h, in_w, &zh, &zw, st))) return rc;
    if (h->cfg.projection_dim > 0) {
        ConvCall pin(B, zh, zw, h->C, h->D, 1, 1, 0, VQAE_PAD_NONE);
        return vqae_conv2d_f32(&pin.a, h->buf[0], h->pin_w, h->pin_b, nullptr, z, st);
    }
    VQAE_HIP_CHECK(hipMemcpyAsync(z, h->buf[0], (size_t)B * zh * zw * h->C * 4, hipMemcpyDeviceToDevice, st));
    return VQAE_OK;
}

extern "C" int vqae_decode(vqae_handle* h, const float* q, int B, int qh, int qw, int layout, float* out, void* stream) {
    if (h) g_dt = h->cfg.compute_dtype;
    hipStream_t st = (hipStream_t)stream;
    VQAE_REQUIRE(h && q && out, VQAE_ERR_INVALID, "vqae_decode: null pointer");
    VQAE_REQUIRE(h->has_decoder, VQAE_ERR_INVALID, "vqae_decode: handle was created without decoder.* tensors");
    VQAE_REQUIRE(B >= 0 && qh >= 1 && qw >= 1, VQAE_ERR_INVALID, "vqae_decode: bad shape");
    if (int rcd = check_device(h)) return rcd;
    if (B == 0) return VQAE_OK;
    int rc;
    if ((rc = ensure_workspace(h, B, qh << h->cfg.n_down, qw << h->cfg.n_down))) return rc;
    if (layout == VQAE_LAYOUT_NCHW) {
        if ((rc = vqae_nchw_to_nhwc_f32(q, B, h->C, qh, qw, h->buf[0], st))) return rc;
    } else {
        VQAE_HIP_CHECK(hipMemcpyAsync(h->buf[0], q, (size_t)B * qh * qw * h->C * 4, hipMemcpyDeviceToDevice, st));
    }
    return run_decoder_convs(h, B, qh, qw, layout, out, st);
}

extern "C" int vqae_decode_indices(vqae_handle* h, const void* idx, int idx_dtype, int B, int qh, int qw, int layout,
                                   float* out, void* stream) {
    if (h) g_dt = h->cfg.compute_dtype;
    hipStream_t st = (hipStream_t)stream;
    VQAE_REQUIRE(h && idx && out, VQAE_ERR_INVALID, "vqae_decode_indices: null pointer");
    VQAE_REQUIRE(h->has_decoder && h->embed, VQAE_ERR_INVALID, "vqae_decode_indices: handle needs decoder.* tensors and a codebook");
    VQAE_REQUIRE(B >= 0 && qh >= 1 && qw >= 1, VQAE_ERR_INVALID, "vqae_decode_indices: bad shape");
    if (int rcd = check_device(h)) return rcd;
    if (B == 0) return VQAE_OK;
    int rc;
    if ((rc = ensure_workspace(h, B, qh << h->cfg.n_down, qw << h->cfg.n_down))) return rc;
    const int64_t rows = (int64_t)B * qh * qw;
    if (h->cfg.projection_dim > 0) {
        if ((rc = vqae_embed_code_f32(idx, idx_dtype, h->embed, rows, h->K, h->D, h->buf[1], st))) return rc;
        ConvCall pout(B, qh, qw, h->D, h->C, 1, 1, 0, VQAE_PAD_NONE);
        if ((rc = vqae_conv2d_f32(&pout.a, h->buf[1], h->pout_w, h->pout_b, nullptr, h->buf[0], st))) return rc;
    } else {
        if ((rc = vqae_embed_code_f32(idx, idx_dtype, h->embed, rows, h->K, h->D, h->buf[0], st))) return rc;
    }
    return run_decoder_convs(h, B, qh, qw, layout, out, st);
}

extern "C" int vqae_block_count(const vqae_handle* h, int side) {
    if (!h) return 0;
    return (int)(side == 0 ? h->enc.size() : h->dec.size());
}

extern "C" int vqae_run_blocks(vqae_handle* h, int side, int first, int count, const float* x, int B, int in_h, int in_w,
                               float* y, int* out_h, int* out_w, void* stream) {
    if (h) g_dt = h->cfg.compute_dtype;
    hipStream_t st = (hipStream_t)stream;
    VQAE_REQUIRE(h && x && y, VQAE_ERR_INVALID, "vqae_run_blocks: null pointer");
    VQAE_REQUIRE(side == 0 || side == 1, VQAE_ERR_INVALID, "vqae_run_blocks: side %d", side);
    std::vector<Block>& v = side == 0 ? h->enc : h->dec;
    VQAE_REQUIRE(first >= 0 && count >= 1 && (size_t)first + (size_t)count <= v.size(), VQAE_ERR_INVALID,
                 "vqae_run_blocks: blocks [%d, %d) of %zu", first, first + count, v.size());
    VQAE_REQUIRE(B >= 0 && in_h >= 1 && in_w >= 1, VQAE_ERR_INVALID, "vqae_run_blocks: bad shape");
    if (int rcd = check_device(h)) return rcd;
    int H = in_h, W = in_w;
    if (B == 0) return VQAE_OK;
    size_t need = 0;
    {
        double hh = in_h, ww = in_w;
        for (int i = first; i < first + count; ++i) {
            const Block& b = v[i];
            VQAE_REQUIRE(b.mode != MODE_DOWN || (((int)hh % 2 == 0) && ((int)ww % 2 == 0)), VQAE_ERR_INVALID,
                         "vqae_run_blocks: odd input size at a 'down' block");
            const size_t wide = (size_t)std::max(std::max(b.cin, b.cout), b.br) * (b.mode == MODE_UP ? 4 : 1);
            need = std::max(need, (size_t)B * (size_t)hh * (size_t)ww * wide);
            if (b.mode == MODE_DOWN) { hh /= 2; ww /= 2; } else if (b.mode == MODE_UP) { hh *= 2; ww *= 2; }
        }
    }
    int rc;
    if ((rc = ensure_bufs(h, need))) return rc;
    if (h->cfg.block_kind == VQAE_BLOCK_MBCONV)
        return vqae::fail(VQAE_ERR_UNSUPPORTED, "vqae_run_blocks: Fixup blocks only");
    VQAE_HIP_CHECK(hipMemcpyAsync(h->buf[0], x, (size_t)B * in_h * in_w * v[first].cin * 4, hipMemcpyDeviceToDevice, st));
    h->t1_ready = false;
    for (int i = first; i < first + count; ++i)
        if ((rc = run_block(h, v[i], i + 1 < first + count ? &v[i + 1] : nullptr, B, H, W, st))) return rc;
    h->t1_ready = false;
    VQAE_HIP_CHECK(hipMemcpyAsync(y, h->buf[0], (size_t)B * H * W * v[first + count - 1].cout * 4, hipMemcpyDeviceToDevice, st));
    if (out_h) *out_h = H;
    if (out_w) *out_w = W;
    return VQAE_OK;
}

extern "C" int vqae_forward(vqae_handle* h, const float* x, int B, int in_h, int in_w, int layout, float* out, void* idx,
                            int idx_dtype, float* loss, void* stream) {
    if (h) g_dt = h->cfg.compute_dtype;
    hipStream_t st = (hipStream_t)stream;
    VQAE_REQUIRE(h && x && out, VQAE_ERR_INVALID, "vqae_forward: null pointer");
    VQAE_REQUIRE(h->has_encoder && h->has_decoder, VQAE_ERR_INVALID, "vqae_forward: handle needs encoder.* and decoder.* tensors");
    int rc = check_geometry(h, B, in_h, in_w);
    if (rc) return rc;
    if (B == 0) return VQAE_OK;
    if ((rc = ensure_workspace(h, B, in_h, in_w))) return rc;
    int zh, zw;
    if ((rc = run_encoder_convs(h, x, layout == VQAE_LAYOUT_NCHW ? 1 : 0, B, in_h, in_w, &zh, &zw, st))) return rc;
    void* idx_out = idx;
    int dt = idx_dtype;
    if (!idx_out) { idx_out = h->idx_scratch; dt = VQAE_IDX_I32; }
    if ((rc = run_vq(h, B, zh, zw, idx_out, dt, loss ? loss : h->loss_scratch, st))) return rc;
    return run_decoder_convs(h, B, zh, zw, layout, out, st);
}

extern "C" double vqae_flops_per_patch(const vqae_handle* h, int in_h, int in_w, int encoder, int decoder) {
    if (!h) return 0.0;
    double fl = 0.0;
    auto blocks = [&](const std::vector<Block>& v, double H, double W) {
        for (const Block& b : v) {
            if (b.kind == VQAE_BLOCK_MBCONV) {
                const double k2 = b.mode == MODE_SAME ? 9.0 : 4.0;
                fl += 2.0 * H * W * (double)b.cin * b.br;
                if (b.mode == MODE_DOWN) {
                    fl += 2.0 * (H / 2) * (W / 2) * (k2 * b.br + (double)b.br * b.cout + 4.0 * b.cin * b.cout);
                    H /= 2; W /= 2;
                } else if (b.mode == MODE_UP) {
                    fl += 2.0 * H * W * 4.0 * b.cin * b.cout;
                    H *= 2; W *= 2;
                    fl += 2.0 * H * W * ((double)b.br + (double)b.br * b.cout);
                } else {
                    fl += 2.0 * H * W * (k2 * b.br + (double)b.br * b.cout + (b.wskip ? (double)b.cin * b.cout : 0.0));
                }
                continue;
            }
            if (b.mode == MODE_SAME) {
                fl += 2.0 * H * W * ((double)b.cin * b.br + 9.0 * b.br * b.br + (double)b.br * b.cout);
            } else if (b.mode == MODE_DOWN) {
                fl += 2.0 * H * W * (double)b.cin * b.br;
                H /= 2; W /= 2;
                fl += 2.0 * H * W * (4.0 * b.br * b.br + (double)b.br * b.cout + 4.0 * b.cin * b.cout);
            } else {
                fl += 2.0 * H * W * (double)b.cin * b.br;
                H *= 2; W *= 2;
                fl += 2.0 * H * W * ((double)b.br * b.br + (double)b.br * b.cout + (double)b.cin * b.cout);
            }
        }
        return std::pair<double, double>(H, W);
    };
    if (encoder) {
        fl += 2.0 * in_h * in_w * 27.0 * h->cfg.stem;
        auto hw = blocks(h->enc, in_h, in_w);
        if (h->cfg.projection_dim > 0) fl += 2.0 * hw.first * hw.second * 2.0 * h->C * h->D;
    }
    if (decoder) {
        blocks(h->dec, in_h >> h->cfg.n_down, in_w >> h->cfg.n_down);
        fl += 2.0 * in_h * in_w * 27.0 * h->cfg.stem;
    }
    return fl;
}
```

Baseline: 4101 patches/s.

## Emulate fp32 Winograd trunk GEMMs with 3-way bf16 split MFMA at C=128

Adds a split-precision path for the C=128 Winograd F(4,3) trunk kernel. Activations and weights are decomposed into three bf16 planes (hi/mid/lo) and multiplied with bf16 MFMA instructions using six cross-products, replacing the fp32 16x16x4 and 32x32x2-style MFMAs in both the Winograd-domain GEMM and the fused 1x1 tail GEMMs. Pre-split weight copies are generated at load time and the feature is on by default. This trades higher-throughput bf16 matrix ops for extra conversion ALU work and a different LDS layout, while aiming to keep near-fp32 accuracy.

```diff
diff --git a/2d-vq-ae-2_amd/csrc/conv_wino43.hip b/2d-vq-ae-2_amd/csrc/conv_wino43.hip
--- a/2d-vq-ae-2_amd/csrc/conv_wino43.hip
+++ b/2d-vq-ae-2_amd/csrc/conv_wino43.hip
@@ -4,6 +4,8 @@
 
 typedef float f32x16 __attribute__((ext_vector_type(16)));
 typedef float f32x4 __attribute__((ext_vector_type(4)));
+typedef __bf16 bf16x4 __attribute__((ext_vector_type(4)));
+typedef __bf16 bf16x8 __attribute__((ext_vector_type(8)));
 using vqae::elu_act;
 using vqae::lds_barrier;
 
@@ -14,6 +16,9 @@
     const float* __restrict__ w1n;
     float* xio;
     float* y2;
+    const float* __restrict__ Us;
+    const float* __restrict__ w3s;
+    const float* __restrict__ w1ns;
     int H, M;
     int stag, first_gen;
     float act_a, act_b, t_scale, t_b4, n_b1a, n_b1b, n_b2a, n_b2b;
@@ -39,6 +44,9 @@
     static constexpr int MI = PXH / ((NWV / WN) * 32);
     static constexpr int V_BYTES = 6 * TILES * LDT * 4, T_BYTES = PXH * LDT * 4;
     static constexpr int LDS_BYTES = V_BYTES > T_BYTES ? V_BYTES : T_BYTES;
+    static constexpr int LDVB = 3 * C + 8, KC = C / 32, KS2 = C / 16;
+    static constexpr int VS_BYTES = 6 * TILES * LDVB * 2;
+    static constexpr int LDS_SPLIT = VS_BYTES > T_BYTES ? VS_BYTES : T_BYTES;
     static_assert(TILES == 2 * TC && RP == TC && PXH / RP == 16 && MI * NI == 4, "geometry");
 };
 #ifndef W43_RD
@@ -53,6 +61,15 @@
 constexpr int EARLY = W43_EARLY;
 constexpr int RD = W43_RD;
 constexpr int RT = 3;
+
+__device__ __forceinline__ void split3(const f32x4& v, bf16x4 (&h)[3]) {
+    h[0] = __builtin_convertvector(v, bf16x4);
+    const f32x4 r1 = v - __builtin_convertvector(h[0], f32x4);
+    h[1] = __builtin_convertvector(r1, bf16x4);
+    const f32x4 r2 = r1 - __builtin_convertvector(h[1], f32x4);
+    h[2] = __builtin_convertvector(r2, bf16x4);
+}
+__device__ __forceinline__ bf16x8 as_bf8(const f32x4& v) { return __builtin_bit_cast(bf16x8, v); }
 
 __device__ __forceinline__ f32x4 fma4(const f32x4& a, float s, const f32x4& c) {
     return __builtin_elementwise_fma(a, f32x4{s, s, s, s}, c);
@@ -71,12 +88,13 @@
 
 template <int N> struct IC { static constexpr int value = N; };
 
-template <int C, int TAIL>
+template <int C, int TAIL, bool SPLIT>
 __global__ __launch_bounds__((W43Cfg<C>::NT), (W43Cfg<C>::NT == 512 ? 1 : 2))
 void wino43_trunk_kernel(const W43K p) {
     using K = W43Cfg<C>;
     constexpr int W = K::W, LDT = K::LDT, KG = K::KG, KS = K::KS, TILES = K::TILES, TC = K::TC, NS = K::NS, C4 = K::C4, RP = K::RP;
     constexpr int MI = K::MI, NI = K::NI, WN = K::WN;
+    constexpr int LDVB = K::LDVB, KC = K::KC, KS2 = K::KS2;
     extern __shared__ __attribute__((aligned(16))) float lds[];
     const int tid = threadIdx.x;
     const int lane = tid & 63;
@@ -149,17 +167,30 @@
     };
     auto columns = [&](int s) __attribute__((always_inline)) {
         float* const dst = lds + (s * TC + tj) * LDT + 4 * cg;
+        __bf16* const dsb = reinterpret_cast<__bf16*>(lds) + (s * TC + tj) * LDVB + 4 * cg;
+        auto put = [&](int nu, const f32x4& v) __attribute__((always_inline)) {
+            if constexpr (SPLIT) {
+                bf16x4 h[3];
+                split3(v, h);
+#pragma unroll
+                for (int pl = 0; pl < 3; ++pl) *reinterpret_cast<bf16x4*>(dsb + nu * TILES * LDVB + pl * C) = h[pl];
+            } else {
+                *reinterpret_cast<f32x4*>(dst + nu * TILES * LDT) = v;
+            }
+        };
         const f32x4 t1 = fma4(w[2], -4.f, w[4]), t2 = fma4(w[1], -4.f, w[3]);
         const f32x4 t3 = w[4] - w[2], t4 = w[3] - w[1];
-        *reinterpret_cast<f32x4*>(dst + 0 * TILES * LDT) = fma4(w[0], 4.f, fma4(w[2], -5.f, w[4]));
-        *reinterpret_cast<f32x4*>(dst + 1 * TILES * LDT) = t1 + t2;
-        *reinterpret_cast<f32x4*>(dst + 2 * TILES * LDT) = t1 - t2;
-        *reinterpret_cast<f32x4*>(dst + 3 * TILES * LDT) = fma4(t4, 2.f, t3);
-        *reinterpret_cast<f32x4*>(dst + 4 * TILES * LDT) = fma4(t4, -2.f, t3);
-        *reinterpret_cast<f32x4*>(dst + 5 * TILES * LDT) = fma4(w[1], 4.f, fma4(w[3], -5.f, w[5]));
+        put(0, fma4(w[0], 4.f, fma4(w[2], -5.f, w[4])));
+        put(1, t1 + t2);
+        put(2, t1 - t2);
+        put(3, fma4(t4, 2.f, t3));
+        put(4, fma4(t4, -2.f, t3));
+        put(5, fma4(w[1], 4.f, fma4(w[3], -5.f, w[5])));
     };
 
     const float* const ub = p.U + ns * (KG * 512);
+    const float* const ubs = p.Us + ns * (KC * 1536);
+    const __bf16* const vbs = reinterpret_cast<const __bf16*>(lds) + (16 * tg + li) * LDVB + 8 * q;
     const unsigned wl = 16u * lane;
     const float* const bfrag = lds + (16 * tg + li) * LDT + 4 * q;
 
@@ -199,55 +230,9 @@
         }
 #endif
         __builtin_amdgcn_sched_barrier(0);
-        int64_t uoff = (int64_t)xi * 6 * (C * C);
-        asm volatile("" : "+s"(uoff));
-        const float* const ux = ub + uoff;
-#define WB(s) (((s) / KG) * (C * C) + 512 * ((s) % KG))
-        f32x4 wq[RD][2];
-#pragma unroll
-        for (int s = 0; s < RD; ++s) {
-            wq[s][0] = ldg(ux + WB(s), wl);
-            wq[s][1] = ldg(ux + WB(s) + 256, wl);
-        }
-        STAMP(1 + 5 * xi);
-#if defined(W43_PRIO) && W43_PRIO == 1
-        __builtin_amdgcn_s_setprio(0);
-#elif defined(W43_PRIO) && W43_PRIO == 2
-        __builtin_amdgcn_s_setprio(3);
-#endif
-        lds_barrier();
-        STAMP(2 + 5 * xi);
         f32x4 Z[4][2];
-#pragma unroll
-        for (int b = 0; b < 4; ++b) { Z[b][0] = f32x4{0.f, 0.f, 0.f, 0.f}; Z[b][1] = f32x4{0.f, 0.f, 0.f, 0.f}; }
         f32x4 acc[2][2];
-        f32x4 bq[2];
-        bq[0] = *reinterpret_cast<const f32x4*>(bfrag);
-#pragma unroll
-        for (int nu = 0; nu < 6; ++nu) {
-            const int st = nu & 1;
-            acc[st][0] = f32x4{0.f, 0.f, 0.f, 0.f};
-            acc[st][1] = f32x4{0.f, 0.f, 0.f, 0.f};
-#pragma unroll
-            for (int kg = 0; kg < KG; ++kg) {
-                const int s = KG * nu + kg;
-                if (s + 1 < 6 * KG)
-                    bq[(s + 1) & 1] = *reinterpret_cast<const f32x4*>(bfrag + ((s + 1) / KG) * TILES * LDT + 16 * ((s + 1) % KG));
-                const f32x4 wa = wq[s % RD][0], wb = wq[s % RD][1];
-                if (s + RD < 6 * KG) {
-                    wq[s % RD][0] = ldg(ux + WB(s + RD), wl);
-                    wq[s % RD][1] = ldg(ux + WB(s + RD) + 256, wl);
-                }
-#pragma unroll
-                for (int j = 0; j < 4; ++j) {
-                    acc[st][0] = __builtin_amdgcn_mfma_f32_16x16x4f32(wa[j], bq[s & 1][j], acc[st][0], 0, 0, 0);
-                    acc[st][1] = __builtin_amdgcn_mfma_f32_16x16x4f32(wb[j], bq[s & 1][j], acc[st][1], 0, 0, 0);
-#ifdef W43_ALT
-                    __builtin_amdgcn_sched_barrier(0);
-#endif
-                }
-                __builtin_amdgcn_sched_barrier(0);
-            }
+        auto fold_nu = [&](int nu) __attribute__((always_inline)) {
 #pragma unroll
             for (int bl = 0; bl < 2; ++bl) {
                 if (nu == 0) Z[0][bl] = Z[0][bl] + acc[0][bl];
@@ -265,8 +250,108 @@
             }
             if (nu == 0 || nu == 2 || nu == 4)
                 asm volatile("" : "+v"(Z[0][0]), "+v"(Z[0][1]), "+v"(Z[1][0]), "+v"(Z[1][1]), "+v"(Z[2][0]), "+v"(Z[2][1]), "+v"(Z[3][0]), "+v"(Z[3][1]));
-        }
+        };
+        if constexpr (SPLIT) {
+            int64_t uoff = (int64_t)xi * 6 * (3 * C * C / 2);
+            asm volatile("" : "+s"(uoff));
+            const float* const ux = ubs + uoff;
+#define WS(s, bl, pl) (((s) / KC) * (3 * C * C / 2) + 1536 * ((s) % KC) + 256 * (3 * (bl) + (pl)))
+#define VB(s, pl) (*reinterpret_cast<const bf16x8*>(vbs + ((s) / KC) * TILES * LDVB + (pl) * C + 32 * ((s) % KC)))
+            f32x4 w0[2][2], w1[2], w2[2];
+#pragma unroll
+            for (int bl = 0; bl < 2; ++bl) {
+                w0[0][bl] = ldg(ux + WS(0, bl, 0), wl);
+                w1[bl] = ldg(ux + WS(0, bl, 1), wl);
+                w2[bl] = ldg(ux + WS(0, bl, 2), wl);
+                w0[1][bl] = ldg(ux + WS(1, bl, 0), wl);
+            }
+            STAMP(1 + 5 * xi);
+            lds_barrier();
+            STAMP(2 + 5 * xi);
+#pragma unroll
+            for (int b = 0; b < 4; ++b) { Z[b][0] = f32x4{0.f, 0.f, 0.f, 0.f}; Z[b][1] = f32x4{0.f, 0.f, 0.f, 0.f}; }
+            bf16x8 vb0 = VB(0, 0), vb1 = VB(0, 1), vb2 = VB(0, 2);
+#pragma unroll
+            for (int nu = 0; nu < 6; ++nu) {
+                const int st = nu & 1;
+                acc[st][0] = f32x4{0.f, 0.f, 0.f, 0.f};
+                acc[st][1] = f32x4{0.f, 0.f, 0.f, 0.f};
+#pragma unroll
+                for (int kc = 0; kc < KC; ++kc) {
+                    const int s = KC * nu + kc, sl = s & 1;
+                    const bool nxt = s + 1 < 6 * KC;
+#define MM(wa, vb) for (int bl = 0; bl < 2; ++bl) acc[st][bl] = __builtin_amdgcn_mfma_f32_16x16x32_bf16(as_bf8(wa[bl]), vb, acc[st][bl], 0, 0, 0)
+                    MM(w1, vb1);
+                    MM(w1, vb0);
+                    if (nxt) for (int bl = 0; bl < 2; ++bl) w1[bl] = ldg(ux + WS(s + 1, bl, 1), wl);
+                    MM(w2, vb0);
+                    if (nxt) for (int bl = 0; bl < 2; ++bl) w2[bl] = ldg(ux + WS(s + 1, bl, 2), wl);
+                    MM(w0[sl], vb2);
+                    if (nxt) vb2 = VB(s + 1, 2);
+                    MM(w0[sl], vb1);
+                    if (nxt) vb1 = VB(s + 1, 1);
+                    MM(w0[sl], vb0);
+                    if (s + 2 < 6 * KC) for (int bl = 0; bl < 2; ++bl) w0[sl][bl] = ldg(ux + WS(s + 2, bl, 0), wl);
+                    if (nxt) vb0 = VB(s + 1, 0);
+#undef MM
+                    __builtin_amdgcn_sched_barrier(0);
+                }
+                fold_nu(nu);
+            }
+#undef WS
+#undef VB
+        } else {
+            int64_t uoff = (int64_t)xi * 6 * (C * C);
+            asm volatile("" : "+s"(uoff));
+            const float* const ux = ub + uoff;
+#define WB(s) (((s) / KG) * (C * C) + 512 * ((s) % KG))
+            f32x4 wq[RD][2];
+#pragma unroll
+            for (int s = 0; s < RD; ++s) {
+                wq[s][0] = ldg(ux + WB(s), wl);
+                wq[s][1] = ldg(ux + WB(s) + 256, wl);
+            }
+            STAMP(1 + 5 * xi);
+#if defined(W43_PRIO) && W43_PRIO == 1
+            __builtin_amdgcn_s_setprio(0);
+#elif defined(W43_PRIO) && W43_PRIO == 2
+            __builtin_amdgcn_s_setprio(3);
+#endif
+            lds_barrier();
+            STAMP(2 + 5 * xi);
+#pragma unroll
+            for (int b = 0; b < 4; ++b) { Z[b][0] = f32x4{0.f, 0.f, 0.f, 0.f}; Z[b][1] = f32x4{0.f, 0.f, 0.f, 0.f}; }
+            f32x4 bq[2];
+            bq[0] = *reinterpret_cast<const f32x4*>(bfrag);
+#pragma unroll
+            for (int nu = 0; nu < 6; ++nu) {
+                const int st = nu & 1;
+                acc[st][0] = f32x4{0.f, 0.f, 0.f, 0.f};
+                acc[st][1] = f32x4{0.f, 0.f, 0.f, 0.f};
+#pragma unroll
+                for (int kg = 0; kg < KG; ++kg) {
+                    const int s = KG * nu + kg;
+                    if (s + 1 < 6 * KG)
+                        bq[(s + 1) & 1] = *reinterpret_cast<const f32x4*>(bfrag + ((s + 1) / KG) * TILES * LDT + 16 * ((s + 1) % KG));
+                    const f32x4 wa = wq[s % RD][0], wb = wq[s % RD][1];
+                    if (s + RD < 6 * KG) {
+                        wq[s % RD][0] = ldg(ux + WB(s + RD), wl);
+                        wq[s % RD][1] = ldg(ux + WB(s + RD) + 256, wl);
+                    }
+#pragma unroll
+                    for (int j = 0; j < 4; ++j) {
+                        acc[st][0] = __builtin_amdgcn_mfma_f32_16x16x4f32(wa[j], bq[s & 1][j], acc[st][0], 0, 0, 0);
+                        acc[st][1] = __builtin_amdgcn_mfma_f32_16x16x4f32(wb[j], bq[s & 1][j], acc[st][1], 0, 0, 0);
+#ifdef W43_ALT
+                        __builtin_amdgcn_sched_barrier(0);
+#endif
+                    }
+                    __builtin_amdgcn_sched_barrier(0);
+                }
+                fold_nu(nu);
+            }
 #undef WB
+        }
         STAMP(3 + 5 * xi);
         __builtin_amdgcn_sched_barrier(0);
         if constexpr (NEXT == 9) {
@@ -326,7 +411,19 @@
     float* const trow = T + tj0 * LDT + 4 * cg;
     const int ty = (16 * tg + li) / TC, tx = (16 * tg + li) % TC;
     f32x4 bt[RT][NI];
+    f32x4 bs0[2][NI], bs1[NI], bs2[NI];
     auto tail_prefetch = [&](const float* __restrict__ wsrc) __attribute__((always_inline)) {
+        if constexpr (SPLIT) {
+            const float* b0 = wsrc + (wn * NI) * (KS2 * 768);
+#pragma unroll
+            for (int ni = 0; ni < NI; ++ni) {
+                bs0[0][ni] = ldg(b0 + ni * (KS2 * 768), wl);
+                bs1[ni] = ldg(b0 + ni * (KS2 * 768) + 256, wl);
+                bs2[ni] = ldg(b0 + ni * (KS2 * 768) + 512, wl);
+                bs0[1][ni] = ldg(b0 + ni * (KS2 * 768) + 768, wl);
+            }
+            return;
+        }
         const float* b0 = wsrc + (wn * NI) * (KS * 256);
 #pragma unroll
         for (int u = 0; u < RT; ++u)
@@ -334,6 +431,38 @@
             for (int ni = 0; ni < NI; ++ni) bt[u][ni] = ldg(b0 + ni * (KS * 256) + 256 * u, wl);
     };
     f32x16 acc[MI][NI];
+    auto gemm_tail_split = [&](const float* __restrict__ wsrc) __attribute__((always_inline)) {
+        const float* a0 = T + (wm * MI * 32 + li32) * LDT + 8 * hh;
+        const float* b0 = wsrc + (wn * NI) * (KS2 * 768);
+#pragma unroll
+        for (int ks = 0; ks < KS2; ++ks) {
+            const int sl = ks & 1;
+            bf16x8 x[MI][3];
+#pragma unroll
+            for (int mi = 0; mi < MI; ++mi) {
+                bf16x4 lo[3], hi[3];
+                split3(*reinterpret_cast<const f32x4*>(a0 + mi * 32 * LDT + 16 * ks), lo);
+                split3(*reinterpret_cast<const f32x4*>(a0 + mi * 32 * LDT + 16 * ks + 4), hi);
+#pragma unroll
+                for (int pl = 0; pl < 3; ++pl) x[mi][pl] = __builtin_shufflevector(lo[pl], hi[pl], 0, 1, 2, 3, 4, 5, 6, 7);
+            }
+#define MM(wa, pb) for (int mi = 0; mi < MI; ++mi) for (int ni = 0; ni < NI; ++ni) \
+                acc[mi][ni] = __builtin_amdgcn_mfma_f32_32x32x16_bf16(as_bf8(wa[ni]), x[mi][pb], acc[mi][ni], 0, 0, 0)
+#define RELOAD(dst, k, pl) for (int ni = 0; ni < NI; ++ni) dst[ni] = ldg(b0 + ni * (KS2 * 768) + 768 * (k) + 256 * (pl), wl)
+            MM(bs1, 1);
+            MM(bs1, 0);
+            if (ks + 1 < KS2) RELOAD(bs1, ks + 1, 1);
+            MM(bs2, 0);
+            if (ks + 1 < KS2) RELOAD(bs2, ks + 1, 2);
+            MM(bs0[sl], 2);
+            MM(bs0[sl], 1);
+            MM(bs0[sl], 0);
+            if (ks + 2 < KS2) RELOAD(bs0[sl], ks + 2, 0);
+#undef MM
+#undef RELOAD
+            __builtin_amdgcn_sched_barrier(0);
+        }
+    };
     auto gemm_tail = [&](const float* __restrict__ wsrc) __attribute__((always_inline)) {
 #pragma unroll
         for (int mi = 0; mi < MI; ++mi)
@@ -341,6 +470,10 @@
             for (int ni = 0; ni < NI; ++ni)
 #pragma unroll
                 for (int r = 0; r < 16; ++r) acc[mi][ni][r] = 0.f;
+        if constexpr (SPLIT) {
+            gemm_tail_split(wsrc);
+            return;
+        }
         const float* a0 = T + (wm * MI * 32 + li32) * LDT + 4 * hh;
         const float* b0 = wsrc + (wn * NI) * (KS * 256);
         f32x4 a[2][MI];
@@ -396,7 +529,7 @@
                     for (int e = 0; e < 4; ++e) o[e] = elu_act(Y[2 * hf + a2][b][bl][e] + p.act_a) + p.act_b;
                     *reinterpret_cast<f32x4*>(T + ((2 * ty + a2) * W + 4 * tx + b) * LDT + 32 * ns + 16 * bl + 4 * q) = o;
                 }
-        tail_prefetch(p.w3);
+        tail_prefetch(SPLIT ? p.w3s : p.w3);
         const int64_t pixb = ((int64_t)img * p.H + row0 + 2 * hf) * W + tj0;
         float* xr[4];
 #pragma unroll
@@ -408,13 +541,13 @@
         STAMP(31 + 8 * hf);
         lds_barrier();
         STAMP(32 + 8 * hf);
-        gemm_tail(p.w3);
+        gemm_tail(SPLIT ? p.w3s : p.w3);
         STAMP(33 + 8 * hf);
         if (hf == 0) {
 #pragma unroll
             for (int i = NRES0; i < 16; ++i) res[i] = __builtin_nontemporal_load(reinterpret_cast<const f32x4*>(xr[(RP * i) / W] + ((RP * i) % W) * C));
         }
-        if (TAIL == 2) tail_prefetch(p.w1n);
+        if (TAIL == 2) tail_prefetch(SPLIT ? p.w1ns : p.w1n);
         lds_barrier();
         acc_to_lds();
         lds_barrier();
@@ -435,7 +568,7 @@
         STAMP(35 + 8 * hf);
         if constexpr (TAIL == 2) {
             lds_barrier();
-            gemm_tail(p.w1n);
+            gemm_tail(SPLIT ? p.w1ns : p.w1n);
             STAMP(36 + 8 * hf);
             lds_barrier();
             acc_to_lds();
@@ -456,22 +589,59 @@
     }
 }
 
-__global__ void wino43_weight_kernel(const float* __restrict__ w, int c, float* __restrict__ U) {
-    const int i = blockIdx.x * blockDim.x + threadIdx.x;
-    if (i >= c * c) return;
+__device__ void wino43_u(const float* __restrict__ w, int64_t i, double (&u)[36]) {
     const double G[6][3] = {{0.25, 0, 0}, {-1.0 / 6, -1.0 / 6, -1.0 / 6}, {-1.0 / 6, 1.0 / 6, -1.0 / 6},
                             {1.0 / 24, 1.0 / 12, 1.0 / 6}, {1.0 / 24, -1.0 / 12, 1.0 / 6}, {0, 0, 1}};
     double g[3][3], t[6][3];
     for (int a = 0; a < 3; ++a)
-        for (int b = 0; b < 3; ++b) g[a][b] = (double)w[(int64_t)i * 9 + a * 3 + b];
+        for (int b = 0; b < 3; ++b) g[a][b] = (double)w[i * 9 + a * 3 + b];
     for (int x = 0; x < 6; ++x)
         for (int b = 0; b < 3; ++b) t[x][b] = G[x][0] * g[0][b] + G[x][1] * g[1][b] + G[x][2] * g[2][b];
+    for (int x = 0; x < 6; ++x)
+        for (int y = 0; y < 6; ++y) u[x * 6 + y] = t[x][0] * G[y][0] + t[x][1] * G[y][1] + t[x][2] * G[y][2];
+}
+
+__global__ void wino43_weight_kernel(const float* __restrict__ w, int c, float* __restrict__ U) {
+    const int i = blockIdx.x * blockDim.x + threadIdx.x;
+    if (i >= c * c) return;
+    double u[36];
+    wino43_u(w, i, u);
     const int n = i / c, k = i % c;
     const int64_t fo = ((((int64_t)(n >> 5) * (c / 16) + (k >> 4)) * 2 + ((n >> 4) & 1)) * 64 + ((k >> 2) & 3) * 16 + (n & 15)) * 4 + (k & 3);
     const int64_t cc = (int64_t)c * c;
-    for (int x = 0; x < 6; ++x)
-        for (int y = 0; y < 6; ++y)
-            U[(x * 6 + y) * cc + fo] = (float)(t[x][0] * G[y][0] + t[x][1] * G[y][1] + t[x][2] * G[y][2]);
+    for (int x = 0; x < 36; ++x) U[x * cc + fo] = (float)u[x];
+}
+
+__device__ void split3_f64(double v, __bf16 (&h)[3]) {
+    for (int pl = 0; pl < 3; ++pl) {
+        h[pl] = (__bf16)(float)v;
+        v -= (double)(float)h[pl];
+    }
+}
+
+__global__ void wino43_split_weight_kernel(const float* __restrict__ w, int c, __bf16* __restrict__ U) {
+    const int i = blockIdx.x * blockDim.x + threadIdx.x;
+    if (i >= c * c) return;
+    double u[36];
+    wino43_u(w, i, u);
+    const int n = i / c, k = i % c;
+    const int64_t fo = (((int64_t)(n >> 5) * (c / 32) + (k >> 5)) * 2 + ((n >> 4) & 1)) * 3 * 512 + (((k >> 3) & 3) * 16 + (n & 15)) * 8 + (k & 7);
+    const int64_t cc = (int64_t)c * c;
+    for (int x = 0; x < 36; ++x) {
+        __bf16 h[3];
+        split3_f64(u[x], h);
+        for (int pl = 0; pl < 3; ++pl) U[x * 3 * cc + fo + pl * 512] = h[pl];
+    }
+}
+
+__global__ void split_1x1_kernel(const float* __restrict__ w, int c, __bf16* __restrict__ out) {
+    const int i = blockIdx.x * blockDim.x + threadIdx.x;
+    if (i >= c * c) return;
+    const int n = i / c, k = i % c;
+    __bf16 h[3];
+    split3_f64((double)w[i], h);
+    const int64_t fo = ((int64_t)(n >> 5) * (c / 16) + (k >> 4)) * 3 * 512 + (((k >> 3) & 1) * 32 + (n & 31)) * 8 + (k & 7);
+    for (int pl = 0; pl < 3; ++pl) out[fo + pl * 512] = h[pl];
 }
 
 }
@@ -489,6 +659,24 @@
 }
 
 size_t wino43_weight_floats(int c) { return (size_t)36 * c * c; }
+
+bool wino43_split_supported(int c) { return c == 128; }
+size_t wino43_split_weight_bytes(int c) { return (size_t)36 * c * c * 3 * 2; }
+size_t split_1x1_bytes(int c) { return (size_t)c * c * 3 * 2; }
+
+int wino43_split_weight(const float* w_oihw_dev, int c, void* U_dev, hipStream_t stream) {
+    VQAE_REQUIRE(wino43_split_supported(c), VQAE_ERR_UNSUPPORTED, "wino43_split_weight: C = %d", c);
+    wino43_split_weight_kernel<<<(unsigned)ceil_div(c * c, 256), 256, 0, stream>>>(w_oihw_dev, c, (__bf16*)U_dev);
+    VQAE_LAUNCH_CHECK();
+    return VQAE_OK;
+}
+
+int split_1x1_weight(const float* w_packed_dev, int c, void* out_dev, hipStream_t stream) {
+    VQAE_REQUIRE(wino43_split_supported(c), VQAE_ERR_UNSUPPORTED, "split_1x1_weight: C = %d", c);
+    split_1x1_kernel<<<(unsigned)ceil_div(c * c, 256), 256, 0, stream>>>(w_packed_dev, c, (__bf16*)out_dev);
+    VQAE_LAUNCH_CHECK();
+    return VQAE_OK;
+}
 
 int wino43_transform_weight(const float* w_oihw_dev, int c, float* U_dev, hipStream_t stream) {
     VQAE_REQUIRE(c == 256 || c == 128 || c == 64 || c == 32, VQAE_ERR_UNSUPPORTED, "wino43_transform_weight: C = %d", c);
@@ -497,24 +685,27 @@
     return VQAE_OK;
 }
 
-template <int C>
+template <int C, bool SPLIT>
 static int launch_w43(W43K& k, int64_t M, bool chain, hipStream_t stream) {
     using K = W43Cfg<C>;
-    static bool attr_set = false;
+    constexpr int lds = SPLIT ? K::LDS_SPLIT : K::LDS_BYTES;
+    static bool attr_set[64] = {};
     static int pad = 0;
-    if (!attr_set) {
+    int dev = 0;
+    VQAE_HIP_CHECK(hipGetDevice(&dev));
+    if (dev < 0 || dev >= 64 || !attr_set[dev]) {
 #ifdef W43_TRACE
         pad = getenv("VQAE_W43_LDS_PAD") ? atoi(getenv("VQAE_W43_LDS_PAD")) : 0;
 #endif
-        VQAE_HIP_CHECK(hipFuncSetAttribute((const void*)wino43_trunk_kernel<C, 1>, hipFuncAttributeMaxDynamicSharedMemorySize, K::LDS_BYTES + pad));
-        VQAE_HIP_CHECK(hipFuncSetAttribute((const void*)wino43_trunk_kernel<C, 2>, hipFuncAttributeMaxDynamicSharedMemorySize, K::LDS_BYTES + pad));
-        attr_set = true;
+        VQAE_HIP_CHECK(hipFuncSetAttribute((const void*)wino43_trunk_kernel<C, 1, SPLIT>, hipFuncAttributeMaxDynamicSharedMemorySize, lds + pad));
+        VQAE_HIP_CHECK(hipFuncSetAttribute((const void*)wino43_trunk_kernel<C, 2, SPLIT>, hipFuncAttributeMaxDynamicSharedMemorySize, lds + pad));
+        if (dev >= 0 && dev < 64) attr_set[dev] = true;
     }
     const unsigned grid = (unsigned)(M / (8 * K::W));
     const double flops = 2.0 * (double)M * C * (2.25 * C + C + (chain ? C : 0));
     ProfScope prof(C >= 128 ? PROF_CONV3X3_TRUNK : PROF_NONE, stream, flops);
-    if (chain) wino43_trunk_kernel<C, 2><<<grid, K::NT, K::LDS_BYTES + pad, stream>>>(k);
-    else wino43_trunk_kernel<C, 1><<<grid, K::NT, K::LDS_BYTES + pad, stream>>>(k);
+    if (chain) wino43_trunk_kernel<C, 2, SPLIT><<<grid, K::NT, lds + pad, stream>>>(k);
+    else wino43_trunk_kernel<C, 1, SPLIT><<<grid, K::NT, lds + pad, stream>>>(k);
     prof.done();
     VQAE_LAUNCH_CHECK();
     return VQAE_OK;
@@ -522,7 +713,8 @@
 
 int wino43_trunk_tail(const float* t1, const float* U, const float* w3, float act_a, float act_b, float t_scale, float t_b4,
                       float* xio, const float* w1n, float n_b1a, float n_b1b, float n_b2a, float n_b2b, float* t1_next,
-                      int batch, int h, int w, int c, hipStream_t stream) {
+                      int batch, int h, int w, int c, hipStream_t stream,
+                      const void* Us, const void* w3s, const void* w1ns) {
     if (batch == 0) return VQAE_OK;
     VQAE_REQUIRE(t1 && U && w3 && xio && (!w1n || t1_next), VQAE_ERR_INVALID, "wino43_trunk_tail: null pointer");
     VQAE_REQUIRE(wino43_supported(c, h, w, VQAE_DT_F32), VQAE_ERR_UNSUPPORTED, "wino43_trunk_tail: C = %d, H = %d, W = %d", c, h, w);
@@ -536,11 +728,16 @@
     k.n_b1a = n_b1a; k.n_b1b = n_b1b; k.n_b2a = n_b2a; k.n_b2b = n_b2b;
     static const int stag = getenv("VQAE_W43_STAG") ? atoi(getenv("VQAE_W43_STAG")) : 0;
     k.stag = stag; k.first_gen = 512;
+    if (Us) {
+        VQAE_REQUIRE(wino43_split_supported(c) && w3s && (!w1n || w1ns), VQAE_ERR_INVALID, "wino43_trunk_tail: split form needs C = 128 and its three weights");
+        k.Us = (const float*)Us; k.w3s = (const float*)w3s; k.w1ns = (const float*)w1ns;
+        return launch_w43<128, true>(k, M, w1n != nullptr, stream);
+    }
     switch (c) {
-        case 256: return launch_w43<256>(k, M, w1n != nullptr, stream);
-        case 128: return launch_w43<128>(k, M, w1n != nullptr, stream);
-        case 64: return launch_w43<64>(k, M, w1n != nullptr, stream);
-        default: return launch_w43<32>(k, M, w1n != nullptr, stream);
+        case 256: return launch_w43<256, false>(k, M, w1n != nullptr, stream);
+        case 128: return launch_w43<128, false>(k, M, w1n != nullptr, stream);
+        case 64: return launch_w43<64, false>(k, M, w1n != nullptr, stream);
+        default: return launch_w43<32, false>(k, M, w1n != nullptr, stream);
     }
 }
 
diff --git a/2d-vq-ae-2_amd/csrc/handle.hip b/2d-vq-ae-2_amd/csrc/handle.hip
--- a/2d-vq-ae-2_amd/csrc/handle.hip
+++ b/2d-vq-ae-2_amd/csrc/handle.hip
@@ -24,9 +24,15 @@
 bool wino43_enabled();
 size_t wino43_weight_floats(int c);
 int wino43_transform_weight(const float* w_oihw_dev, int c, float* U_dev, hipStream_t stream);
+bool wino43_split_supported(int c);
+size_t wino43_split_weight_bytes(int c);
+size_t split_1x1_bytes(int c);
+int wino43_split_weight(const float* w_oihw_dev, int c, void* U_dev, hipStream_t stream);
+int split_1x1_weight(const float* w_packed_dev, int c, void* out_dev, hipStream_t stream);
 int wino43_trunk_tail(const float* t1, const float* U, const float* w3, float act_a, float act_b, float t_scale, float t_b4,
                       float* xio, const float* w1n, float n_b1a, float n_b1b, float n_b2a, float n_b2b, float* t1_next,
-                      int batch, int h, int w, int c, hipStream_t stream);
+                      int batch, int h, int w, int c, hipStream_t stream,
+                      const void* Us, const void* w3s, const void* w1ns);
 int wino_trunk_tail(const float* t1, const float* U, const float* w3, float act_a, float act_b, float t_scale, float t_b4,
                     float* xio, const float* w1n, float n_b1a, float n_b1b, float n_b2a, float n_b2b, float* t1_next,
                     int batch, int h, int w, int c, int dtype, hipStream_t stream);
@@ -131,6 +137,7 @@
     float b1a, b1b, b2a, b2b, b3a, b3b, b4, scale, b1c, b1d;
     float *w1, *w2, *w3, *wskip;
     float* wU43 = nullptr;
+    void *wU43s = nullptr, *w1s = nullptr, *w3s = nullptr;
     float* wU = nullptr;
     float *w1f = nullptr, *w3f = nullptr;
     float *w2f = nullptr, *wskf = nullptr;
@@ -175,6 +182,7 @@
     bool fuse_up16 = true;
     bool fuse_up_tail = true;
     bool use_wino = true;
+    bool w43_split = true;
     void* idx_scratch = nullptr;
     size_t idx_scratch_bytes = 0;
     float* se_ws = nullptr;
@@ -247,18 +255,19 @@
     return rc;
 }
 
-int upload_wino43(vqae_handle* h, const float* host, int c, float** out) {
+int upload_wino43(vqae_handle* h, const float* host, int c, bool split, void** out) {
     void* tmp = nullptr;
     const size_t raw = (size_t)c * c * 9 * 4;
     if (hipMalloc(&tmp, raw) != hipSuccess) return vqae::fail(VQAE_ERR_NOMEM, "hipMalloc failed");
     hipError_t e = hipMemcpy(tmp, host, raw, hipMemcpyHostToDevice);
     void* U = nullptr;
-    int rc = (e == hipSuccess) ? dev_alloc(h, vqae::wino43_weight_floats(c) * 4, &U)
+    int rc = (e == hipSuccess) ? dev_alloc(h, split ? vqae::wino43_split_weight_bytes(c) : vqae::wino43_weight_floats(c) * 4, &U)
                                : vqae::fail(VQAE_ERR_HIP, "hipMemcpy failed: %s", hipGetErrorString(e));
-    if (rc == VQAE_OK) rc = vqae::wino43_transform_weight((const float*)tmp, c, (float*)U, nullptr);
+    if (rc == VQAE_OK) rc = split ? vqae::wino43_split_weight((const float*)tmp, c, U, nullptr)
+                                  : vqae::wino43_transform_weight((const float*)tmp, c, (float*)U, nullptr);
     if (rc == VQAE_OK && hipDeviceSynchronize() != hipSuccess) rc = vqae::fail(VQAE_ERR_HIP, "winograd weight transform failed");
     (void)hipFree(tmp);
-    *out = (float*)U;
+    *out = U;
     return rc;
 }
 
@@ -285,11 +294,14 @@
     if ((rc = find(tm, pre + ".branch_conv2.weight", (int64_t)b->br * b->br * k2 * k2, &p))) return rc;
     if ((rc = upload_packed(h, p, b->br, b->br, k2, &b->w2))) return rc;
     b->wU = b->wU43 = b->w1f = b->w3f = nullptr;
+    b->wU43s = b->w1s = b->w3s = nullptr;
     const bool wino = mode == MODE_SAME && cout == cin && h->use_wino &&
                       (h->cfg.compute_dtype == VQAE_DT_F32 ? (cin == 256 || cin == 128 || cin == 64 || cin == 32) : cin == 32);
     if (wino && (rc = upload_wino(h, p, cin, &b->wU))) return rc;
     if (wino && h->cfg.compute_dtype == VQAE_DT_F32 && vqae::wino43_enabled() && vqae::wino43_supported(cin, 8, cin >= 128 ? 32 : (cin == 64 ? 64 : 128), VQAE_DT_F32) &&
-        (rc = upload_wino43(h, p, cin, &b->wU43))) return rc;
+        (rc = upload_wino43(h, p, cin, false, (void**)&b->wU43))) return rc;
+    const bool split = b->wU43 && h->w43_split && vqae::wino43_split_supported(cin);
+    if (split && (rc = upload_wino43(h, p, cin, true, &b->wU43s))) return rc;
     if ((rc = find(tm, pre + ".branch_conv3.weight", (int64_t)cout * b->br, &p))) return rc;
     if ((rc = upload_packed(h, p, cout, b->br, 1, &b->w3))) return rc;
     if (wino || (mode == MODE_SAME && (cin == 128 || cin == 64) && cout == cin)) {
@@ -298,6 +310,10 @@
         if ((rc = dev_alloc(h, (size_t)cin * cin * 4, &f1)) || (rc = dev_alloc(h, (size_t)cin * cin * 4, &f3))) return rc;
         b->w1f = (float*)f1; b->w3f = (float*)f3;
         if ((rc = vqae::wino_frag_weight(b->w1, cin, sk, b->w1f, nullptr)) || (rc = vqae::wino_frag_weight(b->w3, cin, sk, b->w3f, nullptr))) return rc;
+        if (split) {
+            if ((rc = dev_alloc(h, vqae::split_1x1_bytes(cin), &b->w1s)) || (rc = dev_alloc(h, vqae::split_1x1_bytes(cin), &b->w3s))) return rc;
+            if ((rc = vqae::split_1x1_weight(b->w1, cin, b->w1s, nullptr)) || (rc = vqae::split_1x1_weight(b->w3, cin, b->w3s, nullptr))) return rc;
+        }
         VQAE_HIP_CHECK(hipDeviceSynchronize());
     }
     b->w1h = b->w2h = b->w3h = nullptr;
@@ -516,9 +532,11 @@
         }
         const bool chain = next && next->mode == MODE_SAME && next->cin == b.cin && next->cout == b.cin && (!wino || next->w1f);
         if (wino && b.wU43 && vqae::wino43_supported(b.cin, H, W, g_dt)) {
+            const bool split = b.wU43s && (!chain || next->w1s);
             if ((rc = vqae::wino43_trunk_tail(P, b.wU43, b.w3f, b.b3a, b.b3b, b.scale, b.b4, X, chain ? next->w1f : nullptr,
                                               chain ? next->b1a : 0.f, chain ? next->b1b : 0.f, chain ? next->b2a : 0.f,
-                                              chain ? next->b2b : 0.f, chain ? Q : nullptr, B, H, W, b.cin, st))) return rc;
+                                              chain ? next->b2b : 0.f, chain ? Q : nullptr, B, H, W, b.cin, st,
+                                              split ? b.wU43s : nullptr, b.w3s, chain ? next->w1s : nullptr))) return rc;
             if (chain) std::swap(h->buf[1], h->buf[2]);
             h->t1_ready = chain;
             return VQAE_OK;
@@ -823,6 +841,7 @@
     h->fuse_trunk = !(getenv("VQAE_NO_TRUNK_FUSION") && atoi(getenv("VQAE_NO_TRUNK_FUSION")));
     h->up_conv_first = !(getenv("VQAE_NO_UP_REORDER") && atoi(getenv("VQAE_NO_UP_REORDER")));
     h->use_wino = !(getenv("VQAE_NO_WINOGRAD") && atoi(getenv("VQAE_NO_WINOGRAD")));
+    h->w43_split = !(getenv("VQAE_W43_SPLIT") && !atoi(getenv("VQAE_W43_SPLIT")));
     h->fuse_up_tail = !(getenv("VQAE_NO_UP_TAIL_FUSION") && atoi(getenv("VQAE_NO_UP_TAIL_FUSION")));
     h->fuse_down = !(getenv("VQAE_NO_DOWN_FUSION") && atoi(getenv("VQAE_NO_DOWN_FUSION")));
     h->fuse_down16 = !(getenv("VQAE_NO_DOWN16") && atoi(getenv("VQAE_NO_DOWN16")));
```

New measurement: 4221 patches/s, median of 6. 2.9% higher.
